# PJLab-ADG/nr3d_lib

Hardware: AMD Instinct MI355X
Metric: Mpoints/s LoTD fwd+bwd (16-lvl hash) + Mrays/s march+composite, 1 & 8 GPU (higher is better)
Workload: dtype f32; 1 GPU; configs[1]: 16-level Hash LoTD (gen_ngp_cfg: T=2^19, F=2, 6 Dense + 10 Hash), 2^20 points/GPU, fwd(+dy/dx) + dL/dx + dL/dparam, fp32; points_per_gpu=1048576, n_params=12131648, parallelism=single GPU

## Files before the change

include/nr3d_hip.h:

```cpp
#ifndef NR3D_HIP_H
#define NR3D_HIP_H
#include <stdint.h>

#ifdef __cplusplus
extern "C" {
#endif

enum { NR3D_F32 = 0, NR3D_F16 = 1, NR3D_F64 = 2, NR3D_I32 = 3, NR3D_I64 = 4, NR3D_U8 = 5, NR3D_I16 = 6, NR3D_I8 = 7 };

#define NR3D_ABI_VERSION 11

const char *nr3d_last_error(void);
int nr3d_abi_version(void);

enum {
	NR3D_PROF_LOTD_FWD = 0,
	NR3D_PROF_LOTD_FWD_LDS = 1,
	NR3D_PROF_LOTD_CONTRACT_DX = 2,
	NR3D_PROF_LOTD_BIN = 3,
	NR3D_PROF_LOTD_ACCUM = 4,
	NR3D_PROF_MARCH = 5,
	NR3D_PROF_COMPOSITE_FWD = 6,
	NR3D_PROF_COMPOSITE_BWD = 7,
	NR3D_PROF_LOTD_DIRECT = 8,
	NR3D_PROF_COUNT = 9
};
void nr3d_prof_enable(uint32_t mask);
int nr3d_prof_read(int id, double *total_ms, uint32_t *n_intervals, int reset);

enum {
	NR3D_OPT_LOTD_PAIR = 0,
	NR3D_OPT_PAIR_QUAD = 1,
	NR3D_OPT_PAIR_SECOND = 2,
	NR3D_OPT_PAIR_DIRECT = 3,
	NR3D_OPT_PAIR_FIXED = 4,
	NR3D_OPT_FWD_PAIRLANE = 5,
	NR3D_OPT_FWD_SPLIT = 6,
	NR3D_OPT_FWD_LDS_STAGE = 7,
	NR3D_OPT_HVP_LEVELS = 8,
	NR3D_OPT_HVP_PAIRLANE = 9,
	NR3D_OPT_HVP_SPLIT = 10,
	NR3D_OPT_VM_SPLIT = 11,
	NR3D_OPT_CP_DIRECT = 12,
	NR3D_OPT_MARCH_GROUP = 13,
	NR3D_OPT_PACK_SCAN = 14,
	NR3D_OPT_VM_LINES_DIRECT = 15,
	NR3D_OPT_FWD_CELL_MAJOR = 16,
	NR3D_OPT_SORT_WAVE = 17,
	NR3D_OPT_VM_DIRECT = 18,
	NR3D_OPT_DIRECT_FIXED = 19,
	NR3D_OPT_VM_SORTED = 20,
	NR3D_OPT_MLP_X3 = 21,
	NR3D_OPT_COUNT = 22
};
int nr3d_set_option(int id, int64_t value);
int64_t nr3d_get_option(int id);

#define NR3D_LOTD_MAX_LEVELS 32
#define NR3D_LOTD_MAX_DIMS 4
#define NR3D_LOTD_MAX_PSEUDO 256

enum {
	NR3D_LOD_Dense = 0, NR3D_LOD_VectorMatrix = 1, NR3D_LOD_VecZMatXoY = 2, NR3D_LOD_CP = 3,
	NR3D_LOD_CPfast = 4, NR3D_LOD_NPlaneMul = 5, NR3D_LOD_NPlaneSum = 6, NR3D_LOD_Hash = 7
};

typedef struct nr3d_lotd_level {
	uint32_t res[NR3D_LOTD_MAX_DIMS];
	uint32_t n_feats;
	uint32_t type;
	uint32_t size;
	uint32_t offset;
} nr3d_lotd_level_t;

typedef struct nr3d_lotd_meta {
	nr3d_lotd_level_t levels[NR3D_LOTD_MAX_LEVELS];
	uint16_t map_levels[NR3D_LOTD_MAX_PSEUDO];
	uint16_t map_cnt[NR3D_LOTD_MAX_PSEUDO];
	uint32_t n_levels;
	uint32_t n_pseudo_levels;
	uint32_t n_feat_per_pseudo_lvl;
	uint32_t n_dims_to_encode;
	uint32_t n_encoded_dims;
	uint32_t n_params;
	uint32_t interpolation_type;
	uint32_t c_hash_only;
	uint16_t map_col[NR3D_LOTD_MAX_PSEUDO];
} nr3d_lotd_meta_t;

int nr3d_lotd_meta_create(int32_t n_input_dim, uint32_t n_levels, const int32_t *res_multidim,
                          const int32_t *n_feats, const int32_t *types, uint32_t hashmap_size,
                          int use_smooth_step, nr3d_lotd_meta_t *out);

int nr3d_lotd_meta_regroup(const nr3d_lotd_meta_t *meta, uint32_t width, uint32_t max_width, nr3d_lotd_meta_t *out);


int nr3d_lotd_fwd(const nr3d_lotd_meta_t *meta, const void *meta_dev, uint32_t n_points,
                  int x_dtype, int param_dtype, const void *x, const void *params,
                  const int64_t *batch_inds, const int64_t *batch_offsets, uint32_t batch_data_size,
                  int32_t max_level, void *y, int64_t y_sn, int64_t y_se,
                  void *dy_dx, int64_t dydx_sn, int64_t dydx_se, void *stream);

int nr3d_lotd_bwd_dx(const nr3d_lotd_meta_t *meta, uint32_t n_points, int x_dtype, int param_dtype,
                     const void *dL_dy, int64_t dldy_sn, int64_t dldy_se,
                     const void *dy_dx, int64_t dydx_sn, int64_t dydx_se, void *dL_dx,
                     void *dL_dy_T ,
                     void *stream);

uint64_t nr3d_lotd_dparam_workspace_bytes(const nr3d_lotd_meta_t *meta, uint32_t n_points, uint32_t n_batches);
void nr3d_lotd_set_dparam_chunk_log2(int log2_points);
int nr3d_lotd_bwd_dparam(const nr3d_lotd_meta_t *meta, const void *meta_dev, uint32_t n_points,
                         int x_dtype, int param_dtype, const void *dL_dy, int64_t dldy_sn, int64_t dldy_se,
                         const void *x, const void *params, const int64_t *batch_inds,
                         const int64_t *batch_offsets, uint32_t batch_data_size, uint32_t n_batches, int32_t max_level,
                         void *dL_dparam, void *workspace, uint64_t workspace_bytes, void *stream);
int nr3d_lotd_bwd_dparam_levels(const nr3d_lotd_meta_t *meta, const void *meta_dev, uint32_t n_points,
                                int x_dtype, int param_dtype, const void *dL_dy, int64_t dldy_sn, int64_t dldy_se,
                                const void *x, const void *params, const int64_t *batch_inds,
                                const int64_t *batch_offsets, uint32_t batch_data_size, uint32_t n_batches,
                                int32_t min_level, int32_t max_level, void *dL_dparam, void *workspace,
                                uint64_t workspace_bytes, void *stream);

int nr3d_lotd_dLdy_feature_major(uint32_t n_points, uint32_t n_encoded_dims, int grad_dtype, const void *dL_dy,
                                 int64_t g_sn, int64_t g_se, float *out, void *stream);

int nr3d_lotd_half_params_ok(const nr3d_lotd_meta_t *meta, int batched);
int nr3d_lotd_pair_path_ok(const nr3d_lotd_meta_t *meta);
int nr3d_lotd_pair_direct_levels(const nr3d_lotd_meta_t *meta, uint32_t n_points);
uint64_t nr3d_lotd_fwd_lds_levels(const nr3d_lotd_meta_t *meta, uint32_t n_points, uint64_t *by_slab);
int nr3d_lotd_bwd_dparam_typed(const nr3d_lotd_meta_t *meta, const void *meta_dev, uint32_t n_points, int grad_dtype,
                               const void *dL_dy, int64_t g_sn, int64_t g_se, const void *x, int32_t max_level,
                               int out_dtype, int assign, void *dL_dparam, void *workspace, uint64_t workspace_bytes,
                               void *stream);

int nr3d_lotd_bwd_bwd_ddLdy(const nr3d_lotd_meta_t *meta, uint32_t n_points, int x_dtype, int param_dtype,
                            const void *dL_ddLdx, const void *dy_dx, int64_t dydx_sn, int64_t dydx_se,
                            void *dL_ddLdy, int64_t out_sn, int64_t out_se, void *stream);
int nr3d_lotd_bwd_bwd_dparam(const nr3d_lotd_meta_t *meta, const void *meta_dev, uint32_t n_points,
                             int x_dtype, int param_dtype, const void *dL_ddLdx,
                             const void *dL_dy, int64_t dldy_sn, int64_t dldy_se, const void *x,
                             const void *params, const int64_t *batch_inds, const int64_t *batch_offsets,
                             uint32_t batch_data_size, uint32_t n_batches, int32_t max_level, void *dL_dparam,
                             void *workspace, uint64_t workspace_bytes, void *stream);
int nr3d_lotd_bwd_bwd_dx(const nr3d_lotd_meta_t *meta, const void *meta_dev, uint32_t n_points,
                         int x_dtype, int param_dtype, const void *dL_ddLdx,
                         const void *dL_dy, int64_t dldy_sn, int64_t dldy_se, const void *x,
                         const void *params, const int64_t *batch_inds, const int64_t *batch_offsets,
                         uint32_t batch_data_size, int32_t max_level, void *dL_dx, void *stream);
uint64_t nr3d_lotd_bwd_bwd_dx_workspace_bytes(const nr3d_lotd_meta_t *meta, uint32_t n_points);
int nr3d_lotd_bwd_bwd_dx_ws(const nr3d_lotd_meta_t *meta, const void *meta_dev, uint32_t n_points,
                            int x_dtype, int param_dtype, const void *dL_ddLdx,
                            const void *dL_dy, int64_t dldy_sn, int64_t dldy_se, const void *x,
                            const void *params, const int64_t *batch_inds, const int64_t *batch_offsets,
                            uint32_t batch_data_size, int32_t max_level, void *dL_dx, void *workspace,
                            uint64_t workspace_bytes, void *stream);

int nr3d_lotd_grid_index(const nr3d_lotd_meta_t *meta, const void *meta_dev, uint32_t n_points, int x_dtype,
                         const void *x, const int64_t *batch_inds, const int64_t *batch_offsets,
                         uint32_t batch_data_size, int32_t max_level, int64_t *grid_inds, void *stream);

typedef struct nr3d_forest_meta {
	const uint8_t *octree;
	const int32_t *exsum;
	const int16_t *block_ks;
	float world_block_size[3];
	float world_origin[3];
	int32_t resolution[3];
	uint32_t n_trees;
	uint32_t level;
	uint32_t level_poffset;
	int32_t continuity_enabled;
} nr3d_forest_meta_t;

int nr3d_forest_identify(const nr3d_forest_meta_t *forest, uint64_t n, const int16_t *ks, int32_t *block_inds,
                         void *stream);

int nr3d_lotd_forest_fwd(const nr3d_lotd_meta_t *meta, const void *meta_dev, const nr3d_forest_meta_t *forest,
                         uint32_t n_points, const float *x, const void *params, int param_dtype ,
                         const int64_t *block_inds,
                         const int64_t *block_offsets, uint32_t batch_data_size, int32_t max_level, float *y,
                         int64_t y_sn, int64_t y_se, float *dy_dx, int64_t d_sn, int64_t d_se, void *stream);

uint64_t nr3d_lotd_forest_dparam_workspace_bytes(const nr3d_lotd_meta_t *meta, uint32_t n_points, uint32_t n_trees);
int nr3d_lotd_forest_bwd_dparam(const nr3d_lotd_meta_t *meta, const void *meta_dev, const nr3d_forest_meta_t *forest,
                                uint32_t n_points, const float *dL_ddLdx, const float *dL_dy, const float *x,
                                const void *params, int param_dtype, const int64_t *block_inds, const int64_t *block_offsets,
// ... 255 lines not shown
```

nr3d_lib_amd/_abi.py:

```python
ABI_VERSION = 11
SIGNATURES = {
    'nr3d_abi_version': ('int', []),
    'nr3d_alpha_to_vw_backward': ('int', ['uint32_t', 'uint64_t', 'ptr', 'ptr', 'ptr', 'ptr', 'float', 'float', 'ptr', 'ptr']),
    'nr3d_alpha_to_vw_forward': ('int', ['uint32_t', 'uint64_t', 'ptr', 'ptr', 'float', 'float', 'ptr', 'ptr', 'ptr', 'ptr']),
    'nr3d_arange_num_steps': ('int', ['uint32_t', 'int', 'ptr', 'ptr', 'ptr', 'double', 'ptr', 'ptr']),
    'nr3d_forest_identify': ('int', ['ptr', 'uint64_t', 'ptr', 'ptr', 'ptr']),
    'nr3d_forest_ray_marching_count': ('int', ['ptr', 'uint32_t', 'ptr', 'ptr', 'ptr', 'ptr', 'ptr', 'ptr', 'ptr', 'ptr', 'ptr', 'ptr', 'float', 'float', 'float', 'uint32_t', 'ptr', 'ptr', 'ptr', 'ptr']),
    'nr3d_forest_ray_marching_emit': ('int', ['ptr', 'uint32_t', 'ptr', 'ptr', 'ptr', 'ptr', 'ptr', 'ptr', 'ptr', 'ptr', 'ptr', 'ptr', 'float', 'float', 'float', 'ptr', 'ptr', 'ptr', 'ptr', 'ptr', 'ptr', 'ptr']),
    'nr3d_get_option': ('int64_t', ['int']),
    'nr3d_interleave_linstep': ('int', ['uint32_t', 'int', 'ptr', 'ptr', 'ptr', 'double', 'double', 'ptr', 'ptr', 'ptr']),
    'nr3d_last_error': ('str', []),
    'nr3d_lotd_bwd_bwd_ddLdy': ('int', ['ptr', 'uint32_t', 'int', 'int', 'ptr', 'ptr', 'int64_t', 'int64_t', 'ptr', 'int64_t', 'int64_t', 'ptr']),
    'nr3d_lotd_bwd_bwd_dparam': ('int', ['ptr', 'ptr', 'uint32_t', 'int', 'int', 'ptr', 'ptr', 'int64_t', 'int64_t', 'ptr', 'ptr', 'ptr', 'ptr', 'uint32_t', 'uint32_t', 'int32_t', 'ptr', 'ptr', 'uint64_t', 'ptr']),
    'nr3d_lotd_bwd_bwd_dx': ('int', ['ptr', 'ptr', 'uint32_t', 'int', 'int', 'ptr', 'ptr', 'int64_t', 'int64_t', 'ptr', 'ptr', 'ptr', 'ptr', 'uint32_t', 'int32_t', 'ptr', 'ptr']),
    'nr3d_lotd_bwd_bwd_dx_workspace_bytes': ('uint64_t', ['ptr', 'uint32_t']),
    'nr3d_lotd_bwd_bwd_dx_ws': ('int', ['ptr', 'ptr', 'uint32_t', 'int', 'int', 'ptr', 'ptr', 'int64_t', 'int64_t', 'ptr', 'ptr', 'ptr', 'ptr', 'uint32_t', 'int32_t', 'ptr', 'ptr', 'uint64_t', 'ptr']),
    'nr3d_lotd_bwd_dparam': ('int', ['ptr', 'ptr', 'uint32_t', 'int', 'int', 'ptr', 'int64_t', 'int64_t', 'ptr', 'ptr', 'ptr', 'ptr', 'uint32_t', 'uint32_t', 'int32_t', 'ptr', 'ptr', 'uint64_t', 'ptr']),
    'nr3d_lotd_bwd_dparam_levels': ('int', ['ptr', 'ptr', 'uint32_t', 'int', 'int', 'ptr', 'int64_t', 'int64_t', 'ptr', 'ptr', 'ptr', 'ptr', 'uint32_t', 'uint32_t', 'int32_t', 'int32_t', 'ptr', 'ptr', 'uint64_t', 'ptr']),
    'nr3d_lotd_bwd_dparam_typed': ('int', ['ptr', 'ptr', 'uint32_t', 'int', 'ptr', 'int64_t', 'int64_t', 'ptr', 'int32_t', 'int', 'int', 'ptr', 'ptr', 'uint64_t', 'ptr']),
    'nr3d_lotd_bwd_dx': ('int', ['ptr', 'uint32_t', 'int', 'int', 'ptr', 'int64_t', 'int64_t', 'ptr', 'int64_t', 'int64_t', 'ptr', 'ptr', 'ptr']),
    'nr3d_lotd_dLdy_feature_major': ('int', ['uint32_t', 'uint32_t', 'int', 'ptr', 'int64_t', 'int64_t', 'ptr', 'ptr']),
    'nr3d_lotd_dparam_workspace_bytes': ('uint64_t', ['ptr', 'uint32_t', 'uint32_t']),
    'nr3d_lotd_forest_bwd_bwd_dx': ('int', ['ptr', 'ptr', 'ptr', 'uint32_t', 'ptr', 'ptr', 'ptr', 'ptr', 'int', 'ptr', 'ptr', 'uint32_t', 'int32_t', 'ptr', 'ptr']),
    'nr3d_lotd_forest_bwd_dparam': ('int', ['ptr', 'ptr', 'ptr', 'uint32_t', 'ptr', 'ptr', 'ptr', 'ptr', 'int', 'ptr', 'ptr', 'uint32_t', 'int32_t', 'ptr', 'ptr', 'uint64_t', 'ptr']),
    'nr3d_lotd_forest_dparam_workspace_bytes': ('uint64_t', ['ptr', 'uint32_t', 'uint32_t']),
    'nr3d_lotd_forest_fwd': ('int', ['ptr', 'ptr', 'ptr', 'uint32_t', 'ptr', 'ptr', 'int', 'ptr', 'ptr', 'uint32_t', 'int32_t', 'ptr', 'int64_t', 'int64_t', 'ptr', 'int64_t', 'int64_t', 'ptr']),
    'nr3d_lotd_fwd': ('int', ['ptr', 'ptr', 'uint32_t', 'int', 'int', 'ptr', 'ptr', 'ptr', 'ptr', 'uint32_t', 'int32_t', 'ptr', 'int64_t', 'int64_t', 'ptr', 'int64_t', 'int64_t', 'ptr']),
    'nr3d_lotd_fwd_lds_levels': ('uint64_t', ['ptr', 'uint32_t', 'ptr']),
    'nr3d_lotd_grid_index': ('int', ['ptr', 'ptr', 'uint32_t', 'int', 'ptr', 'ptr', 'ptr', 'uint32_t', 'int32_t', 'ptr', 'ptr']),
    'nr3d_lotd_half_params_ok': ('int', ['ptr', 'int']),
    'nr3d_lotd_meta_create': ('int', ['int32_t', 'uint32_t', 'ptr', 'ptr', 'ptr', 'uint32_t', 'int', 'ptr']),
    'nr3d_lotd_meta_regroup': ('int', ['ptr', 'uint32_t', 'uint32_t', 'ptr']),
    'nr3d_lotd_mlp_forward': ('int', ['ptr', 'ptr', 'uint64_t', 'ptr', 'ptr', 'int', 'int32_t', 'ptr', 'ptr', 'ptr', 'int64_t', 'uint32_t', 'ptr']),
    'nr3d_lotd_mlp_forward_ok': ('int', ['ptr', 'ptr']),
    'nr3d_lotd_pair_direct_levels': ('int', ['ptr', 'uint32_t']),
    'nr3d_lotd_pair_path_ok': ('int', ['ptr']),
    'nr3d_lotd_set_dparam_chunk_log2': ('void', ['int']),
    'nr3d_march_composite_bwd': ('int', ['uint32_t', 'ptr', 'ptr', 'ptr', 'ptr', 'ptr', 'float', 'float', 'int', 'ptr', 'ptr', 'ptr', 'ptr', 'ptr', 'ptr', 'ptr', 'ptr', 'ptr', 'ptr', 'uint64_t', 'ptr', 'ptr']),
    'nr3d_march_composite_fwd': ('int', ['uint32_t', 'ptr', 'ptr', 'ptr', 'ptr', 'ptr', 'ptr', 'ptr', 'int', 'float', 'float', 'float', 'uint32_t', 'ptr', 'ptr', 'ptr', 'ptr', 'ptr', 'ptr', 'uint64_t', 'uint64_t', 'ptr', 'ptr', 'ptr', 'ptr', 'ptr', 'ptr', 'ptr', 'ptr', 'uint64_t', 'ptr', 'float', 'float', 'int', 'ptr', 'ptr', 'ptr', 'ptr', 'ptr', 'ptr']),
    'nr3d_march_finish_rays': ('int', ['uint32_t', 'ptr', 'ptr', 'ptr', 'ptr', 'ptr', 'ptr']),
    'nr3d_march_finish_samples': ('int', ['uint64_t', 'ptr', 'ptr', 'ptr', 'ptr', 'ptr', 'ptr', 'ptr', 'ptr', 'ptr']),
    'nr3d_mark_pack_boundaries': ('int', ['uint64_t', 'int', 'ptr', 'ptr', 'ptr']),
    'nr3d_merge_pack_union': ('int', ['uint32_t', 'ptr', 'ptr', 'uint32_t', 'ptr', 'ptr', 'ptr', 'ptr', 'ptr', 'ptr', 'ptr', 'ptr', 'ptr', 'ptr', 'ptr', 'ptr']),
    'nr3d_mlp_backward': ('int', ['ptr', 'uint64_t', 'ptr', 'int64_t', 'int64_t', 'ptr', 'int64_t', 'ptr', 'ptr', 'int64_t', 'int64_t', 'ptr', 'ptr', 'ptr']),
    'nr3d_mlp_backward_backward': ('int', ['ptr', 'uint64_t', 'ptr', 'int64_t', 'int64_t', 'ptr', 'int64_t', 'ptr', 'int64_t', 'int64_t', 'ptr', 'ptr', 'int64_t', 'ptr', 'ptr']),
    'nr3d_mlp_backward_backward_ok': ('int', ['ptr']),
    'nr3d_mlp_backward_packed_floats': ('uint64_t', ['ptr']),
    'nr3d_mlp_forward': ('int', ['ptr', 'uint64_t', 'ptr', 'int64_t', 'int64_t', 'ptr', 'ptr', 'int64_t', 'ptr']),
    'nr3d_mlp_half_backward': ('int', ['ptr', 'uint64_t', 'ptr', 'int64_t', 'int64_t', 'ptr', 'int64_t', 'ptr', 'ptr', 'int64_t', 'int64_t', 'ptr', 'ptr', 'ptr']),
    'nr3d_mlp_half_backward_packed_bytes': ('uint64_t', ['ptr']),
    'nr3d_mlp_half_forward': ('int', ['ptr', 'uint64_t', 'ptr', 'int64_t', 'int64_t', 'ptr', 'ptr', 'int64_t', 'ptr']),
    'nr3d_mlp_half_pack': ('int', ['ptr', 'ptr', 'ptr', 'ptr', 'int', 'ptr']),
    'nr3d_mlp_half_packed_bytes': ('uint64_t', ['ptr']),
    'nr3d_mlp_pack': ('int', ['ptr', 'ptr', 'ptr', 'ptr', 'int', 'ptr']),
    'nr3d_mlp_packed_floats': ('uint64_t', ['ptr']),
    'nr3d_occ_apply_max': ('int', ['uint64_t', 'float', 'ptr', 'ptr', 'ptr']),
    'nr3d_occ_scatter_max': ('int', ['uint64_t', 'ptr', 'ptr', 'ptr', 'uint64_t', 'ptr', 'ptr', 'uint32_t', 'ptr', 'ptr']),
    'nr3d_octree_mark_consecutive_segments': ('int', ['uint32_t', 'ptr', 'ptr', 'ptr', 'ptr', 'ptr', 'ptr']),
    'nr3d_order_gather_inputs': ('int', ['uint32_t', 'ptr', 'ptr', 'ptr', 'ptr', 'ptr', 'ptr', 'ptr', 'ptr']),
    'nr3d_order_move_rows': ('int', ['uint32_t', 'ptr', 'int', 'ptr', 'uint32_t', 'ptr', 'ptr', 'uint32_t', 'ptr', 'ptr']),
    'nr3d_pack_composite_bwd': ('int', ['uint32_t', 'ptr', 'ptr', 'ptr', 'ptr', 'ptr', 'ptr', 'float', 'float', 'int', 'ptr', 'ptr', 'ptr', 'ptr', 'ptr', 'ptr', 'ptr', 'ptr', 'ptr', 'ptr']),
    'nr3d_pack_composite_fwd': ('int', ['uint32_t', 'ptr', 'ptr', 'ptr', 'ptr', 'ptr', 'float', 'float', 'int', 'ptr', 'ptr', 'ptr', 'ptr', 'ptr']),
    'nr3d_pack_infos_from_n': ('int', ['uint32_t', 'ptr', 'ptr', 'ptr', 'ptr', 'ptr']),
    'nr3d_packed_binary': ('int', ['uint32_t', 'uint64_t', 'uint32_t', 'uint32_t', 'int', 'ptr', 'ptr', 'ptr', 'int', 'int', 'ptr', 'ptr']),
    'nr3d_packed_diff': ('int', ['uint32_t', 'uint64_t', 'uint32_t', 'int', 'ptr', 'ptr', 'ptr', 'ptr', 'int', 'int', 'ptr', 'ptr']),
    'nr3d_packed_invert_cdf': ('int', ['uint32_t', 'ptr', 'ptr', 'ptr', 'ptr', 'uint32_t', 'ptr', 'ptr', 'ptr']),
    'nr3d_packed_scan': ('int', ['uint32_t', 'uint64_t', 'uint32_t', 'int', 'ptr', 'ptr', 'int', 'int', 'int', 'int', 'ptr', 'ptr']),
    'nr3d_packed_searchsorted': ('int', ['uint32_t', 'int', 'ptr', 'ptr', 'ptr', 'uint32_t', 'ptr', 'ptr', 'ptr']),
    'nr3d_packed_sort': ('int', ['uint32_t', 'uint64_t', 'int', 'ptr', 'ptr', 'ptr', 'ptr']),
    'nr3d_packed_sum': ('int', ['uint32_t', 'uint64_t', 'uint32_t', 'int', 'ptr', 'ptr', 'ptr', 'ptr']),
    'nr3d_permuto_bwd': ('int', ['ptr', 'uint32_t', 'int', 'ptr', 'int64_t', 'int64_t', 'ptr', 'ptr', 'ptr', 'ptr', 'ptr', 'ptr', 'uint32_t', 'int32_t', 'uint32_t', 'ptr', 'ptr', 'ptr']),
    'nr3d_permuto_bwd_bwd_input': ('int', ['ptr', 'uint32_t', 'int', 'ptr', 'ptr', 'int64_t', 'int64_t', 'ptr', 'ptr', 'ptr', 'ptr', 'ptr', 'ptr', 'uint32_t', 'int32_t', 'ptr', 'int64_t', 'int64_t', 'ptr', 'ptr']),
    'nr3d_permuto_fwd': ('int', ['ptr', 'uint32_t', 'int', 'ptr', 'ptr', 'ptr', 'ptr', 'ptr', 'ptr', 'uint32_t', 'int32_t', 'ptr', 'int64_t', 'int64_t', 'ptr']),
    'nr3d_permuto_meta_create': ('int', ['int32_t', 'int32_t', 'uint32_t', 'ptr', 'ptr', 'ptr', 'ptr']),
    'nr3d_permuto_supported_n_input_dims': ('int', ['ptr']),
    'nr3d_prof_enable': ('void', ['uint32_t']),
    'nr3d_prof_read': ('int', ['int', 'ptr', 'ptr', 'int']),
    'nr3d_prune_compact_packs': ('int', ['uint32_t', 'ptr', 'ptr', 'ptr', 'ptr', 'ptr', 'ptr', 'ptr', 'ptr']),
    'nr3d_prune_compact_samples': ('int', ['uint32_t', 'ptr', 'ptr', 'ptr', 'ptr', 'ptr', 'ptr', 'ptr', 'ptr', 'ptr', 'ptr', 'ptr', 'ptr', 'ptr']),
    'nr3d_ray_marching_cache_bytes': ('uint64_t', ['uint32_t', 'uint32_t']),
    'nr3d_ray_marching_count': ('int', ['uint32_t', 'ptr', 'ptr', 'ptr', 'ptr', 'ptr', 'ptr', 'ptr', 'int', 'float', 'float', 'float', 'uint32_t', 'int', 'ptr', 'uint32_t', 'ptr', 'ptr', 'ptr', 'ptr', 'uint64_t', 'ptr']),
    'nr3d_ray_marching_count_finished': ('int', ['uint32_t', 'ptr', 'ptr', 'ptr', 'ptr', 'ptr', 'ptr', 'ptr', 'int', 'float', 'float', 'float', 'uint32_t', 'int', 'ptr', 'uint32_t', 'ptr', 'ptr', 'ptr', 'ptr', 'ptr', 'ptr', 'uint64_t', 'ptr']),
    'nr3d_ray_marching_emit': ('int', ['uint32_t', 'ptr', 'ptr', 'ptr', 'ptr', 'ptr', 'ptr', 'ptr', 'int', 'float', 'float', 'float', 'int', 'ptr', 'uint32_t', 'ptr', 'ptr', 'ptr', 'ptr', 'ptr', 'ptr', 'ptr', 'uint32_t', 'ptr']),
    'nr3d_ray_marching_emit_finished': ('int', ['uint32_t', 'ptr', 'ptr', 'int', 'ptr', 'uint32_t', 'ptr', 'ptr', 'uint32_t', 'ptr', 'ptr', 'ptr', 'ptr', 'ptr', 'ptr', 'ptr', 'ptr', 'ptr']),
    'nr3d_sample_step_count': ('int', ['uint32_t', 'ptr', 'ptr', 'uint32_t', 'float', 'float', 'float', 'ptr', 'ptr']),
    'nr3d_sample_step_emit': ('int', ['uint32_t', 'ptr', 'ptr', 'float', 'float', 'float', 'ptr', 'ptr', 'ptr', 'ptr']),
    'nr3d_sample_step_segments': ('int', ['uint32_t', 'ptr', 'ptr', 'ptr', 'ptr', 'ptr', 'uint32_t', 'float', 'float', 'float', 'int', 'ptr', 'ptr', 'ptr', 'ptr', 'ptr', 'ptr', 'ptr']),
    'nr3d_scan_tmp_bytes': ('uint64_t', ['uint64_t']),
# ... 11 lines not shown
```

nr3d_lib_amd/_hip.py:

```python
import ctypes as C
import os
import subprocess
import threading

import torch

from nr3d_lib_amd import _abi

_PKG = os.path.dirname(os.path.abspath(__file__))
LIB_PATH = os.path.join(_PKG, "libnr3d_hip.so")
ABI_VERSION = _abi.ABI_VERSION
CSRC = os.path.join(_PKG, "csrc")

F32, F16, F64, I32, I64, U8, I16, I8 = range(8)
DTYPE_CODE = {
    torch.float32: F32, torch.float16: F16, torch.float64: F64, torch.int32: I32, torch.int64: I64,
    torch.uint8: U8, torch.bool: U8, torch.int16: I16, torch.int8: I8,
}

_lib = None
_lock = threading.Lock()


def build(verbose=False, jobs=None):
# ... 53 lines not shown
    if missing:
        raise RuntimeError(f"nr3d_lib_amd: {LIB_PATH} does not export {missing} (stale build? `make -C nr3d_lib_amd/csrc`)")


POISON = os.environ.get("NR3D_POISON_EMPTY", "0") == "1"


def _poison(t):
    if t.numel() == 0:
        return t
    if t.dtype.is_floating_point:
        t.fill_(float("nan"))
    elif t.dtype == torch.bool:
        t.fill_(True)
    else:
        t.fill_(-0x54545455 if t.dtype in (torch.int32, torch.int64) else 0x2B)
    return t


def empty(*args, **kwargs):
    t = torch.empty(*args, **kwargs)
    return _poison(t) if POISON else t


def empty_like(x, **kwargs):
    t = torch.empty_like(x, **kwargs)
    return _poison(t) if POISON else t


def check(rc):
    if rc != 0:
        raise RuntimeError(lib().nr3d_last_error().decode())


PROF_IDS = dict(lotd_fwd=0, lotd_fwd_lds=1, lotd_contract_dx=2, lotd_bin=3, lotd_accum=4, march=5, composite_fwd=6,
                composite_bwd=7, lotd_direct=8)


def prof_enable(*names):
    mask = 0
    for n in names:
        mask |= 1 << PROF_IDS[n]
    lib().nr3d_prof_enable(C.c_uint32(mask))


def prof_read(name, reset=True):
    ms, n = C.c_double(0.0), C.c_uint32(0)
    check(lib().nr3d_prof_read(C.c_int(PROF_IDS[name]), C.byref(ms), C.byref(n), C.c_int(1 if reset else 0)))
    return float(ms.value), int(n.value)


OPTION_IDS = dict(lotd_pair=0, pair_quad=1, pair_second=2, pair_direct=3, pair_fixed=4, fwd_pairlane=5, fwd_split=6,
                  fwd_lds_stage=7, hvp_levels=8, hvp_pairlane=9, hvp_split=10, vm_split=11, cp_direct=12, march_group=13,
                  pack_scan=14, vm_lines_direct=15, fwd_cell_major=16, sort_wave=17, vm_direct=18, direct_fixed=19, vm_sorted=20, mlp_x3=21)


def set_option(name, value):
    l = lib()
    check(l.nr3d_set_option(OPTION_IDS[name], -1 if value is None else int(value)))


def get_option(name):
    l = lib()
    return int(l.nr3d_get_option(OPTION_IDS[name]))


class options:

    def __init__(self, **kw):
        self.kw, self.old = kw, {}

    def __enter__(self):
        for k, v in self.kw.items():
            self.old[k] = get_option(k)
            set_option(k, v)
        return self

    def __exit__(self, *a):
        for k, v in self.old.items():
            set_option(k, v)
        return False


def ptr(t):
    if t is None:
        return None
    return t.data_ptr()


_raw_stream = getattr(torch._C, "_cuda_getCurrentRawStream", None)


def stream_of(t):
    if _raw_stream is not None:
        return _raw_stream(t.device.index if t.device.index is not None else torch.cuda.current_device())
    return torch.cuda.current_stream(t.device).cuda_stream


def sort_pairs_u32(keys, values=None, bits=32, n_dev=None):
    pair = isinstance(keys, (list, tuple))
    ks = list(keys) if pair else [keys]
    vs = list(values) if isinstance(values, (list, tuple)) else [values] * len(ks)
    assert len(ks) in (1, 2) and all(k.is_cuda and k.dtype == torch.int32 and k.is_contiguous() and k.shape == ks[0].shape for k in ks)
    assert all(v is None or (v.is_cuda and v.dtype == torch.int32 and v.is_contiguous() and v.shape == ks[0].shape) for v in vs)
    n, dev = ks[0].numel(), ks[0].device
    l = lib()
    l.nr3d_sort_pairs_u32_tmp_bytes.restype = C.c_uint64
# ... 160 lines not shown
```

nr3d_lib_amd/bindings/_lotd.py:

```python
import ctypes as C
import enum

import torch

from .. import _hip as H

MAX_LEVELS, MAX_DIMS, MAX_PSEUDO = 32, 4, 256


class LoDType(enum.IntEnum):
    Dense = 0
    VectorMatrix = 1
    VecZMatXoY = 2
    CP = 3
    CPfast = 4
    NPlaneMul = 5
    NPlaneSum = 6
    Hash = 7


class InterpolationType(enum.IntEnum):
    Linear = 0
    Smoothstep = 1

# ... 345 lines not shown
                                              H.F16 if native else H.F32, max_level, C.byref(mlp_desc._c), H.ptr(mlp_packed), H.ptr(out),
                                              out_cols, out_cols, H.stream_of(input)))
    return out


def lod_bwd(lod_meta, dL_dy, input, params, dy_dx=None, batch_inds=None, batch_offsets=None, batch_data_size=None,
            max_level=None, need_input_grad=None, need_param_grad=None, level_buckets=None, on_bucket=None):
    if isinstance(lod_meta, tuple):
        from . import _forest
        return _forest.lod_bwd(lod_meta, dL_dy, input, params, dy_dx, batch_inds, batch_offsets, batch_data_size, max_level,
                               need_input_grad, need_param_grad)
    m = lod_meta
    N, bds = _check_common("bwd", m, input, params, batch_inds, batch_offsets, batch_data_size)
    E, D = m.n_encoded_dims, m.n_dims_to_encode
    H.require_gpu(dL_dy, dy_dx)
    if dL_dy.dim() != 2 or tuple(dL_dy.shape) != (N, E):
        raise RuntimeError(f"bwd: Expected dL_dy of size [{N}, {E}], got {list(dL_dy.shape)}")
    if dL_dy.dtype != params.dtype:
        raise RuntimeError("bwd: Expected dL_dy and grid to have the same dtype")
    if dy_dx is not None and dy_dx.dtype != input.dtype:
        raise RuntimeError("bwd: Expected x and dy_dx to have the same dtype")
    max_level = m.n_levels if max_level is None else int(max_level)
    need_input_grad = bool(input.requires_grad) if need_input_grad is None else bool(need_input_grad)
    need_param_grad = bool(params.requires_grad) if need_param_grad is None else bool(need_param_grad)
    dev = input.device
    dL_dx = dL_dparam = None
    with H.on_device(dev):
        if need_input_grad and dy_dx is None:
            raise RuntimeError("LoTDEncoding::bwd: need `dy_dx` to comput `dL_dx`.")
        batched = batch_inds is not None or batch_offsets is not None or bds != 0
        nothing = max_level <= -1 or not (need_input_grad or need_param_grad) or N == 0
        native = (_native_half(m, params, batched) and level_buckets is None and USE_BINNED_DPARAM and input.dtype == torch.float32
                  and dL_dy.is_contiguous() and E % 4 == 0 and dL_dy.data_ptr() % 8 == 0 and not nothing
                  and params.shape[0] == m.n_params)
        typed = (not nothing and not batched and level_buckets is None and USE_BINNED_DPARAM
                 and (native or params.dtype == torch.float32) and params.shape[0] == m.n_params
                 and bool(H.lib().nr3d_lotd_pair_path_ok(C.byref(m._cmeta()))))
        if need_input_grad:
            dL_dx = (torch.zeros if nothing else H.empty)((N, D), dtype=torch.float32, device=dev)
        if need_param_grad:
            dL_dparam = (H.empty if typed else torch.zeros)((params.shape[0],), dtype=torch.float16 if native else torch.float32,
                                                                device=dev)
        if nothing:
            if need_param_grad and level_buckets is not None and on_bucket is not None:
                for k, (lo, hi) in enumerate(level_buckets):
                    on_bucket(k, dL_dparam[m.level_offsets[int(lo)]:m.level_offsets[min(int(hi), m.n_levels - 1) + 1]])
            return (_cast(dL_dx, input.dtype), _cast(dL_dparam, params.dtype))
        g32 = dL_dy.detach() if native else _f32c(dL_dy.detach())
        gcode = H.F16 if native else H.F32
        gsn, gse = _strides2(g32)
        st = H.stream_of(input)
        tag = ("dx" if need_input_grad else "") + ("dp" if need_param_grad else "")
        with _Prof(m, f"LoTD{D}-bwd-{tag}", N):
            gT = None
            if need_input_grad and N > 0:
                j, jsn, jse = _jac_view(dy_dx.detach(), N, E, D)
                if (need_param_grad and not batched and USE_BINNED_DPARAM and gse == 1 and gsn == E
                        and g32.data_ptr() % 16 == 0):
                    gT = H.empty((E, N), dtype=torch.float32, device=dev)
                H.check(H.lib().nr3d_lotd_bwd_dx(
                    C.byref(m._cmeta()), H.u32(N), C.c_int(H.F32), C.c_int(gcode), H.ptr(g32), H.i64(gsn),
                    H.i64(gse), H.ptr(j), H.i64(jsn), H.i64(jse), H.ptr(dL_dx), H.ptr(gT), st))
            if need_param_grad and N > 0 and typed:
                ws, wsb = _dparam_workspace(m, N, dev, 1)
                if gT is not None:
                    g32, gsn, gse, gcode = gT, 1, N, H.F32
                H.check(H.lib().nr3d_lotd_bwd_dparam_typed(
                    C.byref(m._cmeta()), H.ptr(m._dev(dev)), H.u32(N), C.c_int(gcode), H.ptr(g32), H.i64(gsn), H.i64(gse),
                    H.ptr(_f32c(input.detach())), H.i32(max_level), C.c_int(H.F16 if native else H.F32), C.c_int(1),
                    H.ptr(dL_dparam), H.ptr(ws), C.c_uint64(wsb), st))
            elif need_param_grad and N > 0:
                x32, (p32, pcode) = _f32c(input.detach()), _ptab(params)
                nbat = _n_batches(m, p32, batch_offsets, batched)
                ws, wsb = _dparam_workspace(m, N, dev, nbat)
                if gT is not None:
                    g32, gsn, gse = gT, 1, N
                if level_buckets is None:
                    H.check(H.lib().nr3d_lotd_bwd_dparam(
                        C.byref(m._cmeta()), H.ptr(m._dev(dev)), H.u32(N), C.c_int(H.F32), C.c_int(pcode),
                        H.ptr(g32), H.i64(gsn), H.i64(gse), H.ptr(x32), H.ptr(p32), H.ptr(batch_inds),
                        H.ptr(batch_offsets), H.u32(bds), H.u32(nbat), H.i32(max_level), H.ptr(dL_dparam), H.ptr(ws),
                        C.c_uint64(wsb), st))
                else:
                    if batched:
                        raise RuntimeError("bwd: level_buckets need non-batched params")
                    if params.dtype != torch.float32:
                        raise RuntimeError("bwd: level_buckets need float params (the slices handed out are the result)")
                    seen = set()
                    for k, (lo, hi) in enumerate(level_buckets):
                        lo, hi = int(lo), min(int(hi), m.n_levels - 1)
                        if lo < 0 or lo > hi or seen & set(range(lo, hi + 1)):
                            raise RuntimeError(f"bwd: bad or overlapping level bucket {(lo, hi)}")
                        seen |= set(range(lo, hi + 1))
                        H.check(H.lib().nr3d_lotd_bwd_dparam_levels(
                            C.byref(m._cmeta()), H.ptr(m._dev(dev)), H.u32(N), C.c_int(H.F32), C.c_int(H.F32),
                            H.ptr(g32), H.i64(gsn), H.i64(gse), H.ptr(x32), H.ptr(p32), None, None, H.u32(0),
                            H.u32(nbat), H.i32(lo), H.i32(min(hi, max_level)), H.ptr(dL_dparam), H.ptr(ws),
                            C.c_uint64(wsb), st))
                        if on_bucket is not None:
                            on_bucket(k, dL_dparam[m.level_offsets[lo]:m.level_offsets[hi + 1]])
    return _cast(dL_dx, input.dtype), _cast(dL_dparam, params.dtype)


def _cast(t, dtype):
    if t is None or t.dtype == dtype:
        return t
    return t.to(dtype)


def lod_bwd_bwd_input(lod_meta, dL_ddLdx, dL_dy, input, params, dy_dx=None, batch_inds=None, batch_offsets=None,
                      batch_data_size=None, max_level=None, need_dLdinput_ddLdoutput=None,
                      need_dLdinput_dparams=None, need_dLdinput_dinput=None):
    if isinstance(lod_meta, tuple):
        from . import _forest
        return _forest.lod_bwd_bwd_input(lod_meta, dL_ddLdx, dL_dy, input, params, dy_dx, batch_inds, batch_offsets,
                                         batch_data_size, max_level, need_dLdinput_ddLdoutput, need_dLdinput_dparams,
                                         need_dLdinput_dinput)
    m = lod_meta
    N, bds = _check_common("bwd_bwd_input", m, input, params, batch_inds, batch_offsets, batch_data_size)
    E, D = m.n_encoded_dims, m.n_dims_to_encode
    H.require_gpu(dL_ddLdx, dL_dy, dy_dx)
    if input.dtype != torch.float32:
        raise RuntimeError("LoTDEncoding: Input type combination not supported. Supported types are: "
# ... 87 lines not shown
```

nr3d_lib_amd/csrc/host_api.hip:

```cpp
#include "common.h"
#include <stdlib.h>
#include <utility>
#include <string.h>
#include <limits>
#include <chrono>
#include <mutex>
#include <vector>

namespace nr3d {

static thread_local char g_err[512] = {0};

char *err_buf() { return g_err; }

int fail(const char *fmt, ...) {
	va_list ap;
	va_start(ap, fmt);
	vsnprintf(g_err, sizeof(g_err), fmt, ap);
	va_end(ap);
	return 1;
}

namespace prof {
uint32_t g_mask = 0;
struct Pair { hipEvent_t a, b; };
static std::mutex g_mu;
static std::vector<Pair> g_done[NR3D_PROF_COUNT];
static std::vector<Pair> g_free;
static Pair g_open[NR3D_PROF_COUNT];
static bool g_is_open[NR3D_PROF_COUNT] = {};

void begin(int id, hipStream_t st) {
	std::lock_guard<std::mutex> lk(g_mu);
	if (id < 0 || id >= NR3D_PROF_COUNT || g_is_open[id]) return;
	Pair p;
	if (!g_free.empty()) { p = g_free.back(); g_free.pop_back(); }
	else if (hipEventCreate(&p.a) != hipSuccess || hipEventCreate(&p.b) != hipSuccess) return;
	if (hipEventRecord(p.a, st) != hipSuccess) return;
	g_open[id] = p; g_is_open[id] = true;
}
void end(int id, hipStream_t st) {
	std::lock_guard<std::mutex> lk(g_mu);
	if (id < 0 || id >= NR3D_PROF_COUNT || !g_is_open[id]) return;
	g_is_open[id] = false;
	if (hipEventRecord(g_open[id].b, st) == hipSuccess) g_done[id].push_back(g_open[id]);
}
}

namespace opt {
static const int64_t kDefault[NR3D_OPT_COUNT] = {
	 1,  1,  1,  1,  1,  1,
	 1,  1,  1,  1,  1,  1,
	 1,  0,  1,  0,  1,  1,
	 1,  1,  1,  1,
};
std::atomic<int64_t> g_val[NR3D_OPT_COUNT] = {1, 1, 1, 1, 1, 1, 1, 1, 1, 1, 1, 1, 1, 0, 1, 0, 1, 1, 1, 1, 1, 1};

#ifdef NR3D_EXPERIMENTS
int64_t experiment_env(const char *name, int64_t dflt) {
	static std::mutex mu;
	static std::vector<std::pair<const char *, int64_t>> seen;
	std::lock_guard<std::mutex> lk(mu);
	for (const auto &kv : seen) if (kv.first == name) return kv.second;
	const char *e = getenv(name);
	const int64_t v = e ? (int64_t)atoll(e) : dflt;
	seen.emplace_back(name, v);
	return v;
}
#endif
}

}

using namespace nr3d;

extern "C" void nr3d_prof_enable(uint32_t mask) { prof::g_mask = mask; }

extern "C" int nr3d_prof_read(int id, double *total_ms, uint32_t *n_intervals, int reset) {
	NR3D_CHECK(id >= 0 && id < NR3D_PROF_COUNT && total_ms && n_intervals, "prof_read: bad argument");
	std::lock_guard<std::mutex> lk(prof::g_mu);
	double sum = 0.0;
	for (const prof::Pair &p : prof::g_done[id]) {
		NR3D_HIP_CHECK(hipEventSynchronize(p.b));
		float ms = 0.0f;
		NR3D_HIP_CHECK(hipEventElapsedTime(&ms, p.a, p.b));
		sum += ms;
	}
	*total_ms = sum;
	*n_intervals = (uint32_t)prof::g_done[id].size();
	if (reset) {
		for (const prof::Pair &p : prof::g_done[id]) prof::g_free.push_back(p);
		prof::g_done[id].clear();
	}
	return 0;
}

extern "C" int nr3d_set_option(int id, int64_t value) {
	NR3D_CHECK(id >= 0 && id < NR3D_OPT_COUNT, "nr3d_set_option: unknown option %d", id);
	opt::g_val[id].store(value < 0 ? opt::kDefault[id] : value, std::memory_order_relaxed);
	return 0;
}
extern "C" int64_t nr3d_get_option(int id) { return (id >= 0 && id < NR3D_OPT_COUNT) ? opt::get(id) : -1; }

extern "C" int nr3d_wait_host_words(const int64_t *words, int n, int64_t sentinel, uint32_t timeout_us) {
	if (!words || n <= 0) return 0;
	const auto t0 = std::chrono::steady_clock::now();
	for (uint32_t spin = 0;; ++spin) {
		bool all = true;
		for (int i = 0; i < n; ++i)
// ... 136 lines not shown
```

nr3d_lib_amd/csrc/lotd.hip:

```cpp
#include "lotd_device.h"
#include <stdlib.h>
#include <vector>
#include <type_traits>
#include <algorithm>

namespace nr3d {
namespace lotd {

template <typename YT> __device__ __forceinline__ void store_nt(YT *p, float v);

template <int D, int G, bool DYDX, bool DH, int ONLY = -1, typename PT = float>
__global__ __launch_bounds__(kBlock) void k_fwd(Sched s, const nr3d_lotd_meta_t *__restrict__ md, uint32_t N,
                                                int32_t max_level, uint32_t smooth, const float *__restrict__ x,
                                                const PT *__restrict__ params, Batch ba, uint32_t vec_ok,
                                                PT *__restrict__ y, int64_t y_sn, int64_t y_se,
                                                float *__restrict__ dydx, int64_t d_sn, int64_t d_se) {
	uint32_t q, chunk;
	if (!decode_block(s, blockIdx.x, q, chunk)) return;
	const uint32_t i = chunk * kBlock + threadIdx.x;
	if (i >= N) return;
	const uint32_t level = meta_level_of(md, q);
	const uint32_t foff0 = meta_cnt_of(md, q) * G;
	const uint32_t out0 = meta_col_of(md, q);

// ... 1149 lines not shown
		if (side == 0u && g0 + pl < N) {
			float *dst = reinterpret_cast<float *>(reinterpret_cast<char *>(partial) + ((size_t)q * N + g0) * 12u + pl * 12u);
			__builtin_nontemporal_store(ox[u], &dst[0]);
			__builtin_nontemporal_store(oy[u], &dst[1]);
			__builtin_nontemporal_store(oz[u], &dst[2]);
		}
	}
}

template <int D>
__global__ __launch_bounds__(kBlock) void k_sum_levels(uint32_t N, uint32_t n_pseudo, const float *__restrict__ partial,
                                                       float *__restrict__ dL_dx) {
	const uint32_t i = blockIdx.x * kBlock + threadIdx.x;
	if (i >= N) return;
	float acc[D];
#pragma unroll
	for (int d = 0; d < D; ++d) acc[d] = 0.0f;
	for (uint32_t q = 0; q < n_pseudo; ++q) {
		const float *src = partial + ((size_t)q * N + i) * D;
#pragma unroll
		for (int d = 0; d < D; ++d) acc[d] += __builtin_nontemporal_load(src + d);
	}
#pragma unroll
	for (int d = 0; d < D; ++d) dL_dx[(size_t)i * D + d] = acc[d];
}


template <int D>
__global__ __launch_bounds__(kBlock) void k_contract_dx(uint32_t N, uint32_t E, const float *__restrict__ dL_dy,
                                                        int64_t g_sn, int64_t g_se, const float *__restrict__ dydx,
                                                        int64_t d_sn, int64_t d_se, float *__restrict__ dL_dx) {
	const uint32_t i = blockIdx.x * kBlock + threadIdx.x;
	if (i >= N) return;
	float acc[D];
#pragma unroll
	for (int d = 0; d < D; ++d) acc[d] = 0.0f;
	const float *gy = dL_dy + (int64_t)i * g_sn;
	const float *jj = dydx + (int64_t)i * d_sn;
#pragma unroll 4
	for (uint32_t e = 0; e < E; ++e) {
		const float g = gy[(int64_t)e * g_se];
		const float *j = jj + (int64_t)e * d_se;
#pragma unroll
		for (int d = 0; d < D; ++d) acc[d] = __fmaf_rn(g, j[d], acc[d]);
	}
#pragma unroll
	for (int d = 0; d < D; ++d) dL_dx[(size_t)i * D + d] = acc[d];
}

template <int D, typename GT>
__global__ __launch_bounds__(kBlock) void k_contract_dx_rowmajor(uint32_t N, uint32_t E, const GT *__restrict__ dL_dy,
                                                                 const float *__restrict__ dydx, int64_t d_sn,
                                                                 int64_t d_se, float *__restrict__ dL_dx,
                                                                 float *__restrict__ dL_dy_T) {
	constexpr int TE = 32;
	__shared__ float tile[TE][kBlock + 1];
	const uint32_t i0 = blockIdx.x * kBlock, i = i0 + threadIdx.x;
	const uint32_t n_here = min((uint32_t)kBlock, N - i0);
	float acc[D];
#pragma unroll
	for (int d = 0; d < D; ++d) acc[d] = 0.0f;
	for (uint32_t e0 = 0; e0 < E; e0 += TE) {
		const uint32_t te = min((uint32_t)TE, E - e0);
		if (te == TE && (E & 3u) == 0u) {
#pragma unroll
			for (uint32_t v = threadIdx.x; v < kBlock * TE / 4; v += kBlock) {
				const uint32_t p = v >> 3, e4 = (v & 7u) * 4u;
				if (p < n_here) {
					float4 t;
					if constexpr (sizeof(GT) == 4) {
						t = *reinterpret_cast<const float4 *>(dL_dy + (size_t)(i0 + p) * E + e0 + e4);
					} else {
						const __half2 *h = reinterpret_cast<const __half2 *>(dL_dy + (size_t)(i0 + p) * E + e0 + e4);
						const float2 a = __half22float2(h[0]), b = __half22float2(h[1]);
						t = make_float4(a.x, a.y, b.x, b.y);
					}
					tile[e4][p] = t.x; tile[e4 + 1][p] = t.y; tile[e4 + 2][p] = t.z; tile[e4 + 3][p] = t.w;
				}
			}
		} else {
			for (uint32_t v = threadIdx.x; v < kBlock * te; v += kBlock) {
				const uint32_t p = v / te, e = v - p * te;
				if (p < n_here) tile[e][p] = to_f32<GT>(dL_dy[(size_t)(i0 + p) * E + e0 + e]);
			}
		}
		__syncthreads();
		if (dL_dy_T && i < N) {
#pragma unroll 8
			for (uint32_t e = 0; e < te; ++e) __builtin_nontemporal_store(tile[e][threadIdx.x], &dL_dy_T[(size_t)(e0 + e) * N + i]);
		}
		if (i < N) {
			const float *jj = dydx + (int64_t)i * d_sn + (int64_t)e0 * d_se;
#pragma unroll 8
			for (uint32_t e = 0; e < te; ++e) {
				const float g = tile[e][threadIdx.x];
				const float *j = jj + (int64_t)e * d_se;
#pragma unroll
				for (int d = 0; d < D; ++d) acc[d] = __fmaf_rn(g, __builtin_nontemporal_load(j + d), acc[d]);
			}
		}
		__syncthreads();
	}
	if (i < N) {
#pragma unroll
		for (int d = 0; d < D; ++d) dL_dx[(size_t)i * D + d] = acc[d];
	}
}

template <int D>
__global__ __launch_bounds__(kBlock) void k_contract_ddLdy(uint32_t N, uint32_t E, const float *__restrict__ v,
                                                           const float *__restrict__ dydx, int64_t d_sn, int64_t d_se,
                                                           float *__restrict__ out, int64_t o_sn, int64_t o_se) {
	const uint32_t i = blockIdx.x * kBlock + threadIdx.x;
	const uint32_t e = blockIdx.y;
	if (i >= N) return;
	const float *j = dydx + (int64_t)i * d_sn + (int64_t)e * d_se;
	float r = 0.0f;
#pragma unroll
	for (int d = 0; d < D; ++d) r = __fmaf_rn(v[(size_t)i * D + d], j[d], r);
	out[(int64_t)i * o_sn + (int64_t)e * o_se] = r;
}

template <int D, int G>
__global__ __launch_bounds__(kBlock) void k_grid_index(Sched s, const nr3d_lotd_meta_t *__restrict__ md, uint32_t N,
                                                       uint32_t E, int32_t max_level, const float *__restrict__ x,
                                                       Batch ba, int64_t *__restrict__ out) {
	uint32_t q, chunk;
	if (!decode_block(s, blockIdx.x, q, chunk)) return;
	const uint32_t i = chunk * kBlock + threadIdx.x;
	if (i >= N) return;
	const uint32_t level = meta_level_of(md, q);
	if ((int32_t)level > max_level) return;
	uint32_t base = 0;
	if (!batch_base(ba, i, base)) return;
	const Lvl L = load_level(md, level);
	const uint32_t foff0 = meta_cnt_of(md, q) * G;
	float xp[D];
#pragma unroll
	for (int d = 0; d < D; ++d) xp[d] = x[(size_t)i * D + d];
	Cell<D> c;
	locate<D>(xp, L, false, c);
	int64_t *dst = out + ((size_t)i * E + (size_t)meta_col_of(md, q)) * (1u << D);
#pragma unroll
	for (uint32_t k = 0; k < (1u << D); ++k) {
		uint32_t p[D];
		corner_pos<D>(c, k, p);
		const uint32_t e = (L.type == NR3D_LOD_Dense) ? entry_dense<D>(L, p) : entry_hash<D>(L, p);
		const uint32_t ind = base + L.off + e * L.F + foff0;
#pragma unroll
		for (int f = 0; f < G; ++f) dst[k + f * (1u << D)] = (int64_t)(uint32_t)(ind + f);
	}
}

static uint32_t sched_mode_default() { const int64_t m = NR3D_XOPT(LOTD_SCHED, 3); return (m < 0 || m > 3) ? 3u : (uint32_t)m; }
static bool sched_exclusive_enabled() { return NR3D_XOPT(LOTD_SCHED_EXCL, 1) != 0; }

static uint32_t level_cost(const nr3d_lotd_meta_t *m, uint32_t q, bool pairlane = false) {
	const nr3d_lotd_level_t &L = m->levels[m->map_levels[q]];
// ... 318 lines not shown
                       bool p_half, const int64_t *batch_inds, const int64_t *batch_offsets, uint32_t batch_data_size,
                       int32_t max_level, void *y, int64_t y_sn, int64_t y_se, void *dy_dx, int64_t d_sn, int64_t d_se,
                       hipStream_t st) {
	uint32_t n_blocks;
	const Batch ba{batch_inds, batch_offsets, batch_data_size, meta->n_params};
	const uint32_t G = meta->n_feat_per_pseudo_lvl;
	const uint32_t elt = p_half ? 2u : 4u;
	const uint32_t vec_ok = (((uintptr_t)params % ((G >= 4 ? 4u : 2u) * elt)) == 0 && batch_offsets == nullptr) ? 1u : 0u;
	const bool dh = meta->c_hash_only != 0;
	prof::Scope ps(NR3D_PROF_LOTD_FWD, st);
	uint64_t grp[4] = {0, 0, 0, 0};
	const bool split = !dh && meta->n_pseudo_levels <= 64u && opt::on(NR3D_OPT_FWD_SPLIT);
	const uint64_t all = meta->n_pseudo_levels >= 64u ? ~0ull : ((1ull << meta->n_pseudo_levels) - 1ull);
	if (split) {
		for (uint32_t q = 0; q < meta->n_pseudo_levels; ++q) {
			const uint32_t t = meta->levels[meta->map_levels[q]].type;
			int k = 0;
			if (t == NR3D_LOD_Dense || t == NR3D_LOD_Hash) k = 1;
			else if (meta->n_dims_to_encode == 3 && t == NR3D_LOD_CP) k = 2;
			else if (meta->n_dims_to_encode == 3 && t == NR3D_LOD_VectorMatrix) k = 3;
			grp[k] |= 1ull << q;
		}
	} else {
		grp[dh ? 1 : 0] = all;
	}
	for (int k = 0; k < 4; ++k) {
		if (!grp[k]) continue;
		const uint64_t skip = (split || meta->n_pseudo_levels <= 64u) ? (all & ~grp[k]) : 0ull;
		const Sched s = make_sched(N, meta, n_blocks, skip);
		if (n_blocks == 0) continue;
		DISPATCH_DG(meta->n_dims_to_encode, G, {
			auto launch = [&](auto kern_f32, auto kern_f16) {
				if (p_half)
					hipLaunchKernelGGL(kern_f16, dim3(n_blocks), dim3(kBlock), 0, st, s, md, N, max_level,
					                   meta->interpolation_type, (const float *)x, (const __half *)params, ba, vec_ok,
					                   (__half *)y, y_sn, y_se, (float *)dy_dx, d_sn, d_se);
				else
					hipLaunchKernelGGL(kern_f32, dim3(n_blocks), dim3(kBlock), 0, st, s, md, N, max_level,
					                   meta->interpolation_type, (const float *)x, (const float *)params, ba, vec_ok,
					                   (float *)y, y_sn, y_se, (float *)dy_dx, d_sn, d_se);
			};
			if (k == 1) { if (dy_dx) NR3D_FWD2(D, true, true, -1); else NR3D_FWD2(D, false, true, -1); }
			else if (k == 0) { if (dy_dx) NR3D_FWD2(D, true, false, -1); else NR3D_FWD2(D, false, false, -1); }
			else if constexpr (D == 3) {
				if (k == 2) { if (dy_dx) NR3D_FWD2(3, true, false, NR3D_LOD_CP); else NR3D_FWD2(3, false, false, NR3D_LOD_CP); }
				else { if (dy_dx) NR3D_FWD2(3, true, false, NR3D_LOD_VectorMatrix); else NR3D_FWD2(3, false, false, NR3D_LOD_VectorMatrix); }
			}
		});
	}
	NR3D_LAUNCH_CHECK();
	return 0;
}

extern "C" int nr3d_lotd_bwd_dx(const nr3d_lotd_meta_t *meta, uint32_t N, int x_dtype, int param_dtype,
                                const void *dL_dy, int64_t g_sn, int64_t g_se, const void *dy_dx, int64_t d_sn,
                                int64_t d_se, void *dL_dx, void *dL_dy_T, void *stream) {
	NR3D_CHECK(meta != nullptr, "LoTD: meta is NULL");
	NR3D_CHECK(x_dtype == NR3D_F32 && (param_dtype == NR3D_F32 || param_dtype == NR3D_F16), "LoTD::bwd_dx: f32 x, f32 / f16 dL_dy");
	if (N == 0) return 0;
	NR3D_CHECK(dL_dy && dy_dx && dL_dx, "LoTDEncoding::bwd: need `dy_dx` to comput `dL_dx`.");
	const uint32_t E = meta->n_encoded_dims;
	const bool g_half = param_dtype == NR3D_F16;
	const bool row_major = (g_se == 1 && g_sn == (int64_t)E && ((uintptr_t)dL_dy % (g_half ? 8 : 16)) == 0);
	NR3D_CHECK(dL_dy_T == nullptr || row_major, "LoTD::bwd_dx: dL_dy_T needs a contiguous, 16-byte aligned [N, E] dL_dy");
	NR3D_CHECK(!g_half || (row_major && (E & 3u) == 0u), "LoTD::bwd_dx: half dL_dy must be a contiguous [N, E] tensor, E % 4 == 0");
	prof::Scope ps(NR3D_PROF_LOTD_CONTRACT_DX, (hipStream_t)stream);
	DISPATCH_D(meta->n_dims_to_encode, {
		if (row_major && g_half)
			hipLaunchKernelGGL((k_contract_dx_rowmajor<D, __half>), dim3(div_up(N, kBlock)), dim3(kBlock), 0, (hipStream_t)stream, N, E,
			                   (const __half *)dL_dy, (const float *)dy_dx, d_sn, d_se, (float *)dL_dx, (float *)dL_dy_T);
		else if (row_major)
			hipLaunchKernelGGL((k_contract_dx_rowmajor<D, float>), dim3(div_up(N, kBlock)), dim3(kBlock), 0, (hipStream_t)stream, N, E,
			                   (const float *)dL_dy, (const float *)dy_dx, d_sn, d_se, (float *)dL_dx, (float *)dL_dy_T);
		else
			hipLaunchKernelGGL(k_contract_dx<D>, dim3(div_up(N, kBlock)), dim3(kBlock), 0, (hipStream_t)stream, N, E,
			                   (const float *)dL_dy, g_sn, g_se, (const float *)dy_dx, d_sn, d_se, (float *)dL_dx);
	});
	NR3D_LAUNCH_CHECK();
	return 0;
}

static int launch_bwd_dparam(bool second, const nr3d_lotd_meta_t *meta, const void *meta_dev, uint32_t N,
                             const void *dL_ddLdx, const void *dL_dy, int64_t g_sn, int64_t g_se, const void *x,
                             const void *params, const int64_t *batch_inds, const int64_t *batch_offsets,
                             uint32_t batch_data_size, uint32_t n_batches, int32_t max_level, void *dL_dparam,
                             void *workspace, uint64_t workspace_bytes, void *stream, int32_t min_level = 0, bool p_half = false) {
	if (N == 0 || max_level <= -1 || min_level > max_level) return 0;
	NR3D_CHECK(dL_dy && x && params && dL_dparam, "LoTD::bwd: NULL tensor pointer");
	const bool batched = batch_inds || batch_offsets || batch_data_size;
	if (workspace && (!batched || n_batches > 0)) {
		bool handled = false;
		const Batch bb{batch_inds, batch_offsets, batch_data_size, meta->n_params};
		if (int rc = dparam_binned(second, meta, meta_dev, N, (const float *)dL_ddLdx, (const float *)dL_dy, g_sn, g_se,
		                           (const float *)x, (const float *)params, bb, batched ? n_batches : 1u, max_level,
		                           (float *)dL_dparam, workspace, workspace_bytes, (hipStream_t)stream, handled, nullptr,
		                           min_level, false, false, false, p_half))
			return rc;
		if (handled) return 0;
	}
	uint32_t n_blocks;
	const Sched s = make_sched(N, meta, n_blocks);
	const Batch ba{batch_inds, batch_offsets, batch_data_size, meta->n_params};
	const auto md = (const nr3d_lotd_meta_t *)meta_dev;
	const bool dh = meta->c_hash_only != 0;
	DISPATCH_DG(meta->n_dims_to_encode, meta->n_feat_per_pseudo_lvl, {
		auto launch = [&](auto kern, auto *tab) {
			hipLaunchKernelGGL(kern, dim3(n_blocks), dim3(kBlock), 0, (hipStream_t)stream, s, md, N, min_level, max_level,
			                   meta->interpolation_type, (const float *)dL_ddLdx, (const float *)dL_dy, g_sn, g_se,
			                   (const float *)x, tab, ba, (float *)dL_dparam);
		};
		const float *pf = (const float *)params;
		const __half *ph = (const __half *)params;
		if (dh || !p_half) {
			if (second) { if (dh) launch(k_bwd_dparam<D, G, true, true>, pf); else launch(k_bwd_dparam<D, G, true, false>, pf); }
			else        { if (dh) launch(k_bwd_dparam<D, G, false, true>, pf); else launch(k_bwd_dparam<D, G, false, false>, pf); }
		} else {
			if (second) launch(k_bwd_dparam<D, G, true, false, __half>, ph); else launch(k_bwd_dparam<D, G, false, false, __half>, ph);
		}
	});
	NR3D_LAUNCH_CHECK();
	return 0;
}

extern "C" int nr3d_lotd_bwd_dparam(const nr3d_lotd_meta_t *meta, const void *meta_dev, uint32_t N, int x_dtype,
                                    int param_dtype, const void *dL_dy, int64_t g_sn, int64_t g_se, const void *x,
                                    const void *params, const int64_t *batch_inds, const int64_t *batch_offsets,
                                    uint32_t batch_data_size, uint32_t n_batches, int32_t max_level, void *dL_dparam,
                                    void *workspace, uint64_t workspace_bytes, void *stream) {
	if (int rc = check_common(meta, meta_dev, x_dtype, param_dtype, true)) return rc;
	return launch_bwd_dparam(false, meta, meta_dev, N, nullptr, dL_dy, g_sn, g_se, x, params, batch_inds,
	                         batch_offsets, batch_data_size, n_batches, max_level, dL_dparam, workspace, workspace_bytes,
	                         stream, 0, param_dtype == NR3D_F16);
}

extern "C" int nr3d_lotd_pair_path_ok(const nr3d_lotd_meta_t *meta) { return (meta && pair_applies(meta)) ? 1 : 0; }
extern "C" uint64_t nr3d_lotd_fwd_lds_levels(const nr3d_lotd_meta_t *meta, uint32_t n_points, uint64_t *by_slab) {
	if (by_slab) *by_slab = 0;
	if (!meta || !pairlane_enabled() || !pairlane_meta_ok(meta)) return 0;
	return fwd_lds_levels(meta, n_points, 0x7fffffff, by_slab);
}

extern "C" int nr3d_lotd_pair_direct_levels(const nr3d_lotd_meta_t *meta, uint32_t n_points) {
	return (meta && pair_applies(meta)) ? (int)pair_direct_levels(meta, n_points) : 0;
}

extern "C" int nr3d_lotd_bwd_dparam_typed(const nr3d_lotd_meta_t *meta, const void *meta_dev, uint32_t N, int grad_dtype,
                                          const void *dL_dy, int64_t g_sn, int64_t g_se, const void *x, int32_t max_level,
                                          int out_dtype, int assign, void *dL_dparam, void *workspace, uint64_t workspace_bytes,
                                          void *stream) {
	if (int rc = check_common(meta, meta_dev, NR3D_F32, NR3D_F32)) return rc;
	NR3D_CHECK((grad_dtype == NR3D_F32 || grad_dtype == NR3D_F16) && (out_dtype == NR3D_F32 || out_dtype == NR3D_F16),
	           "LoTD::bwd_dparam_typed: f32 / f16 only");
	if (N == 0 || max_level <= -1) {
		if (assign && dL_dparam)
			NR3D_HIP_CHECK(hipMemsetAsync(dL_dparam, 0, (size_t)meta->n_params * (out_dtype == NR3D_F16 ? 2 : 4), (hipStream_t)stream));
		return 0;
	}
	NR3D_CHECK(dL_dy && x && dL_dparam && workspace, "LoTD::bwd: NULL tensor pointer");
	bool handled = false;
	const Batch bb{nullptr, nullptr, 0u, meta->n_params};
	if (int rc = dparam_binned(false, meta, meta_dev, N, nullptr, (const float *)dL_dy, g_sn, g_se, (const float *)x, nullptr, bb,
	                           1u, max_level, (float *)dL_dparam, workspace, workspace_bytes, (hipStream_t)stream, handled, nullptr,
	                           0, grad_dtype == NR3D_F16, out_dtype == NR3D_F16, assign != 0))
		return rc;
	NR3D_CHECK(handled, "LoTD::bwd_dparam_typed: the pair-record path does not apply to this meta / workspace");
	return 0;
}

extern "C" int nr3d_lotd_bwd_dparam_levels(const nr3d_lotd_meta_t *meta, const void *meta_dev, uint32_t N, int x_dtype,
                                           int param_dtype, const void *dL_dy, int64_t g_sn, int64_t g_se, const void *x,
                                           const void *params, const int64_t *batch_inds, const int64_t *batch_offsets,
                                           uint32_t batch_data_size, uint32_t n_batches, int32_t min_level,
                                           int32_t max_level, void *dL_dparam, void *workspace, uint64_t workspace_bytes,
                                           void *stream) {
	if (int rc = check_common(meta, meta_dev, x_dtype, param_dtype, true)) return rc;
	NR3D_CHECK(min_level >= 0, "LoTD::bwd: min_level must be >= 0");
	return launch_bwd_dparam(false, meta, meta_dev, N, nullptr, dL_dy, g_sn, g_se, x, params, batch_inds,
	                         batch_offsets, batch_data_size, n_batches, max_level, dL_dparam, workspace, workspace_bytes,
	                         stream, min_level, param_dtype == NR3D_F16);
}

extern "C" void nr3d_lotd_set_dparam_chunk_log2(int log2_points) { set_dparam_chunk_log2(log2_points); }

extern "C" uint64_t nr3d_lotd_dparam_workspace_bytes(const nr3d_lotd_meta_t *meta, uint32_t n_points, uint32_t n_batches) {
	return dparam_workspace_bytes(meta, n_points, n_batches);
}

extern "C" int nr3d_lotd_bwd_bwd_dparam(const nr3d_lotd_meta_t *meta, const void *meta_dev, uint32_t N, int x_dtype,
                                        int param_dtype, const void *dL_ddLdx, const void *dL_dy, int64_t g_sn,
                                        int64_t g_se, const void *x, const void *params, const int64_t *batch_inds,
                                        const int64_t *batch_offsets, uint32_t batch_data_size, uint32_t n_batches,
                                        int32_t max_level, void *dL_dparam, void *workspace, uint64_t workspace_bytes,
                                        void *stream) {
	if (int rc = check_common(meta, meta_dev, x_dtype, param_dtype, true)) return rc;
	NR3D_CHECK(N == 0 || dL_ddLdx != nullptr, "LoTD::bwd_bwd_input: dL_ddLdx is NULL");
	return launch_bwd_dparam(true, meta, meta_dev, N, dL_ddLdx, dL_dy, g_sn, g_se, x, params, batch_inds,
	                         batch_offsets, batch_data_size, n_batches, max_level, dL_dparam, workspace, workspace_bytes,
	                         stream, 0, param_dtype == NR3D_F16);
}

extern "C" int nr3d_lotd_bwd_bwd_ddLdy(const nr3d_lotd_meta_t *meta, uint32_t N, int x_dtype, int param_dtype,
                                       const void *dL_ddLdx, const void *dy_dx, int64_t d_sn, int64_t d_se,
                                       void *dL_ddLdy, int64_t o_sn, int64_t o_se, void *stream) {
	NR3D_CHECK(meta != nullptr, "LoTD: meta is NULL");
	NR3D_CHECK(x_dtype == NR3D_F32 && param_dtype == NR3D_F32, "LoTD::bwd_bwd_ddLdy: f32 only");
	if (N == 0) return 0;
	NR3D_CHECK(dL_ddLdx && dy_dx && dL_ddLdy, "LoTDEncoding::bwd_bwd_input: need `dy_dx` to compute `dL_d(dLdy)`.");
	DISPATCH_D(meta->n_dims_to_encode, {
		hipLaunchKernelGGL(k_contract_ddLdy<D>, dim3(div_up(N, kBlock), meta->n_encoded_dims), dim3(kBlock), 0,
		                   (hipStream_t)stream, N, meta->n_encoded_dims, (const float *)dL_ddLdx,
		                   (const float *)dy_dx, d_sn, d_se, (float *)dL_ddLdy, o_sn, o_se);
	});
	NR3D_LAUNCH_CHECK();
	return 0;
}

template <typename PT>
static int launch_bwd_bwd_dx_t(const nr3d_lotd_meta_t *meta, const void *meta_dev, uint32_t N, int x_dtype, int param_dtype,
                             const void *dL_ddLdx, const void *dL_dy, int64_t g_sn, int64_t g_se, const void *x,
// ... 141 lines not shown
```

nr3d_lib_amd/csrc/lotd_bin.hip:

```cpp
#include "lotd_vm.h"
#include "lotd_sorted.h"
#include <stdlib.h>
#include <type_traits>

#ifndef NR3D_BIN_LDS_KB
#define NR3D_BIN_LDS_KB 72
#define NR3D_BIN_MAX_BP 512
#endif
namespace nr3d {
namespace lotd {

constexpr int kAccThreads = 1024;
constexpr int kLdsDoubles = 16384;
constexpr int kRedSlots = 4;
#ifndef NR3D_BALLOT_RANK_BUCKETS
#define NR3D_BALLOT_RANK_BUCKETS 4
#endif
constexpr uint32_t kBallotRankBuckets = NR3D_BALLOT_RANK_BUCKETS;
constexpr int kMaxPlanLevels = 64;
constexpr uint32_t kMaxBuckets = 8192;
constexpr int kBinLdsDyn = NR3D_BIN_LDS_KB * 1024 + (int)(kMaxBuckets + 1) * 4;

#define DISPATCH_DG_BIN(D_, G_, ...)                                                 \
	do {                                                                             \
// ... 881 lines not shown
		p[k] = flush_target<G>(plan, L, ba, foff0, b, (row0 + (uint32_t)k) * kAccThreads + threadIdx.x, dparam, slot[k]);
		if (!p[k]) slot[k] = 0;
		sum[k] = 0.0f;
	}
#pragma unroll
	for (int k = 0; k < NS; ++k) old[k] = p[k] ? *p[k] : 0.0f;
	for (uint32_t r0 = 0; r0 < R; r0 += NR) {
		float v[NS][NR];
#pragma unroll
		for (int k = 0; k < NS; ++k)
#pragma unroll
			for (int j = 0; j < NR; ++j) v[k][j] = (r0 + j < R) ? part0[(size_t)(r0 + j) * kLdsDoubles + slot[k]] : 0.0f;
#pragma unroll
		for (int k = 0; k < NS; ++k)
#pragma unroll
			for (int j = 0; j < NR; ++j) sum[k] += v[k][j];
	}
#pragma unroll
	for (int k = 0; k < NS; ++k) if (p[k]) *p[k] = old[k] + sum[k];
}

template <int D, int G>
__global__ __launch_bounds__(kAccThreads) void k_reduce_partials(BinPlan plan, const nr3d_lotd_meta_t *__restrict__ md,
                                                                 const uint32_t *__restrict__ rep_g,
                                                                 const uint32_t *__restrict__ item_start, Batch ba,
                                                                 const float *__restrict__ partial,
                                                                 float *__restrict__ dparam) {
	const uint32_t fb = blockIdx.x;
	const uint32_t R = rep_g[fb];
	if (R <= 1) return;
	const bool wide = R <= 4;
	if (wide && blockIdx.y >= kLdsDoubles / kAccThreads / kRedSlots) return;
	uint32_t q = 0;
	while (q + 1 < plan.n_pseudo && plan.bucket_base[q + 1] <= fb) ++q;
	const uint32_t b = fb - plan.bucket_base[q], qg = plan.qmap[q];
	const Lvl L = load_level(md, meta_level_of(md, qg));
	const uint32_t foff0 = meta_cnt_of(md, qg) * G;
	const float *part0 = partial + (size_t)item_start[fb] * kLdsDoubles;
	if (wide) reduce_rows<G, kRedSlots, 4>(plan, L, ba, foff0, b, R, blockIdx.y * kRedSlots, part0, dparam);
	else reduce_rows<G, 1, 8>(plan, L, ba, foff0, b, R, blockIdx.y, part0, dparam);
}

static uint32_t work_units() {
	const int64_t v = NR3D_XOPT(LOTD_ACC_UNITS, 960);
	return (uint32_t)(v < 256 ? 256 : (v > 8192 ? 8192 : v));
}

static int g_chunk_log2 = 0;
void set_dparam_chunk_log2(int lg) { g_chunk_log2 = lg <= 0 ? 0 : (lg < 10 ? 10 : (lg > 24 ? 24 : lg)); }
static uint32_t chunk_points(uint32_t n) {
	const uint32_t chunk = 1u << (g_chunk_log2 ? g_chunk_log2 : 22);
	return n < chunk ? n : chunk;
}

constexpr int kCpThreads = 1024;
constexpr uint32_t kCpMaxItems = 32, kCpLdsBytes = 144 * 1024, kCpReplicas = 128, kCpMaxPairs = 4;
struct CpPlan {
	uint32_t n_items, R, pts_per_rep;
	uint32_t q[kCpMaxItems];
	uint32_t np[kCpMaxItems];
	uint32_t part_off[kCpMaxItems];
};

template <bool SECOND, typename PT>
__global__ __launch_bounds__(kCpThreads) void k_cp_direct(CpPlan cp, const nr3d_lotd_meta_t *__restrict__ md, uint32_t n, uint32_t smooth,
                                                          const float *__restrict__ x, const float *__restrict__ vin_,
                                                          const float *__restrict__ g, int64_t g_sn, int64_t g_se,
                                                          const PT *__restrict__ params, float *__restrict__ partial, uint32_t opt_fix) {
	extern __shared__ __attribute__((aligned(16))) double cp_acc[];
	unsigned long long *cp_fix = reinterpret_cast<unsigned long long *>(cp_acc);
	__shared__ uint32_t s_bound[3];
	const uint32_t r = blockIdx.x, item = blockIdx.y;
	const uint32_t q = cp.q[item], np = cp.np[item], row = 2u * np;
	const Lvl L = load_level(md, meta_level_of(md, q));
	const uint32_t n_acc = L.size * row;
	for (uint32_t t = threadIdx.x; t < n_acc; t += kCpThreads) cp_acc[t] = 0.0;
	if (threadIdx.x < 3) s_bound[threadIdx.x] = 0u;
	__syncthreads();
	const uint32_t foff = meta_cnt_of(md, q) * 2u, col0 = meta_col_of(md, q);
	const auto grid = make_tab(params + L.off + foff);
	const bool vec = (tab_addr(grid) % (2u * tab_elt(grid))) == 0u && (L.F & 1u) == 0u;
	const bool quad = (tab_addr(grid) % (4u * tab_elt(grid))) == 0u && (L.F & 3u) == 0u;
	const uint32_t p_lo = r * cp.pts_per_rep, p_hi = min(n, p_lo + cp.pts_per_rep);
	{
		uint32_t gb = 0u, pb = 0u, vb = 0u;
		for (uint32_t i = p_lo + threadIdx.x; i < p_hi; i += kCpThreads) {
			for (uint32_t f = 0; f < row; ++f) gb = max(gb, __float_as_uint(g[(int64_t)i * g_sn + (int64_t)(col0 + f) * g_se]) & 0x7FFFFFFFu);
			if (SECOND)
#pragma unroll
				for (int d = 0; d < 3; ++d) vb = max(vb, __float_as_uint(vin_[(size_t)i * 3 + d]) & 0x7FFFFFFFu);
		}
		for (uint32_t t = threadIdx.x; t < n_acc; t += kCpThreads)
			pb = max(pb, __float_as_uint((float)grid[(t / row) * L.F + (t % row)]) & 0x7FFFFFFFu);
#pragma unroll
		for (int off = 32; off >= 1; off >>= 1) {
			gb = max(gb, (uint32_t)__shfl_xor((int)gb, off, 64)); pb = max(pb, (uint32_t)__shfl_xor((int)pb, off, 64));
			vb = max(vb, (uint32_t)__shfl_xor((int)vb, off, 64));
		}
		if ((threadIdx.x & 63u) == 0u) { atomicMax(&s_bound[0], gb); atomicMax(&s_bound[1], pb); atomicMax(&s_bound[2], vb); }
	}
	__syncthreads();
	double fscale = 0.0, finv = 0.0;
	bool fix = false;
	{
		const float gmax = __uint_as_float(s_bound[0]), pmax = __uint_as_float(s_bound[1]), vmax = __uint_as_float(s_bound[2]);
		float B = gmax * pmax * pmax;
// ... 514 lines not shown
				hipLaunchKernelGGL((k_bin<D, G, false, NR, false, __half>), dim3(pl.n_blk, pl.n_pseudo), dim3(BP), bin_lds, st, pl, md, n, max_level,
				                   meta->interpolation_type, xc, vc, gc, sn, se, (const __half *)params_, ba, rec, offs);
		}
	} else if (second)
		hipLaunchKernelGGL((k_bin<D, G, true, NR, DH>), dim3(pl.n_blk, pl.n_pseudo), dim3(BP), bin_lds, st, pl, md, n, max_level,
		                   meta->interpolation_type, xc, vc, gc, sn, se, params, ba, rec, offs);
	else
		hipLaunchKernelGGL((k_bin<D, G, false, NR, DH>), dim3(pl.n_blk, pl.n_pseudo), dim3(BP), bin_lds, st, pl, md, n, max_level,
		                   meta->interpolation_type, xc, vc, gc, sn, se, params, ba, rec, offs);
	prof::end(NR3D_PROF_LOTD_BIN, st);
	hipLaunchKernelGGL(k_bucket_totals, dim3(div_up(NB, 4)), dim3(256), 0, st, pl, offs, tot);
	hipLaunchKernelGGL(k_plan_items, dim3(1), dim3(1024), 0, st, NB, pl.n_blk, work_units(), tot, rep, item_start);
	{
		prof::Scope ps(NR3D_PROF_LOTD_ACCUM, st);
		hipLaunchKernelGGL((k_accum<D, G>), dim3(work_units() + NB), dim3(kAccThreads), kLdsDoubles * 8, st, pl, md, rec, offs, rep,
		                   item_start, ba, partial, dparam);
	}
	hipLaunchKernelGGL((k_reduce_partials<D, G>), dim3(NB, kLdsDoubles / kAccThreads), dim3(kAccThreads), 0, st, pl, md, rep, item_start, ba, partial, dparam);
	NR3D_LAUNCH_CHECK();
	return 0;
}

}
}

extern "C" int nr3d_lotd_dLdy_feature_major(uint32_t n_points, uint32_t n_encoded_dims, int grad_dtype, const void *dL_dy,
                                            int64_t g_sn, int64_t g_se, float *out, void *stream) {
	using namespace nr3d;
	using namespace nr3d::lotd;
	NR3D_CHECK(grad_dtype == NR3D_F32 || grad_dtype == NR3D_F16, "dLdy_feature_major: f32 / f16 dL_dy");
	if (n_points == 0 || n_encoded_dims == 0) return 0;
	NR3D_CHECK(dL_dy && out, "dLdy_feature_major: NULL tensor pointer");
	if (grad_dtype == NR3D_F16) launch_transpose<__half>(n_points, n_encoded_dims, (const __half *)dL_dy, g_sn, g_se, out, (hipStream_t)stream);
	else launch_transpose<float>(n_points, n_encoded_dims, (const float *)dL_dy, g_sn, g_se, out, (hipStream_t)stream);
	NR3D_LAUNCH_CHECK();
	return 0;
}

static_assert(sizeof(nr3d_lotd_meta_t) % 4 == 0 && sizeof(nr3d_lotd_meta_t) <= 3584, "the narrowed meta rides in the kernel arguments");
__global__ void k_store_meta(const nr3d_lotd_meta_t m, uint32_t *__restrict__ dst) {
	const uint32_t *src = (const uint32_t *)&m;
	for (uint32_t i = threadIdx.x; i < sizeof(nr3d_lotd_meta_t) / 4; i += blockDim.x) dst[i] = src[i];
}

namespace nr3d {
namespace lotd {

static bool pair_second_enabled() { return opt::on(NR3D_OPT_PAIR_SECOND); }

int dparam_binned(bool second, const nr3d_lotd_meta_t *meta, const void *meta_dev, uint32_t N, const float *dL_ddLdx,
                  const float *dL_dy, int64_t g_sn, int64_t g_se, const float *x, const float *params, const Batch &batch,
                  uint32_t n_batches, int32_t max_level, float *dparam, void *workspace, uint64_t workspace_bytes,
                  hipStream_t st, bool &handled, const ForestDev *forest, int32_t min_level, bool g_half, bool out_half, bool assign,
                  bool p_half) {
	handled = false;
	BinLayout lay;
	const uint32_t nc = chunk_points(N);
	nr3d_lotd_meta_t narrow;
	const bool narrowed = workspace && stage_a_meta(meta, forest != nullptr, narrow);
	if (narrowed) meta = &narrow;
	if (!workspace || !binnable(meta, forest != nullptr) || !layout(meta, nc, n_batches, lay, forest != nullptr)) return 0;
	if (workspace_bytes < lay.total + (narrowed ? kStageAMetaBytes : 0)) return 0;
	handled = true;
	if (narrowed) {
		k_store_meta<<<1, 256, 0, st>>>(narrow, (uint32_t *)((char *)workspace + lay.total));
		NR3D_HIP_CHECK(hipGetLastError());
		meta_dev = (char *)workspace + lay.total;
	}
	const auto md = (const nr3d_lotd_meta_t *)meta_dev;
	const uint32_t D = meta->n_dims_to_encode, G = meta->n_feat_per_pseudo_lvl, E = meta->n_encoded_dims;
	uint32_t *rec = (uint32_t *)workspace;
	uint32_t *offs = (uint32_t *)((char *)workspace + lay.rec_bytes);
	uint32_t *plan_buf = (uint32_t *)((char *)workspace + lay.rec_bytes + lay.offs_bytes);
	float *partial = (float *)((char *)workspace + lay.rec_bytes + lay.offs_bytes + lay.plan_bytes);
	float *gt = (float *)((char *)workspace + lay.rec_bytes + lay.offs_bytes + lay.plan_bytes + lay.part_bytes);
	const bool row_major = (g_se == 1 && g_sn == (int64_t)E && E > 1) || g_half;
	const bool use_pair = !forest && n_batches <= 1 && !batch.inds && !batch.offsets && !batch.data_size && pair_applies(meta) &&
	                      !(second && !pair_second_enabled());
	if ((g_half || out_half) && !use_pair)
		return ::nr3d::fail("LoTD::bwd: half gradients are served natively on the pair-record path only (nr3d_lotd_half_params_ok)");
	const bool assign_now = assign && use_pair && N <= nc && min_level <= 0 && max_level >= (int32_t)meta->n_levels - 1;
	if (assign && !assign_now)
		NR3D_HIP_CHECK(hipMemsetAsync(dparam, 0, (size_t)(n_batches ? n_batches : 1u) * meta->n_params * (out_half ? 2 : 4), st));

	for (uint32_t p0 = 0; p0 < N; p0 += nc) {
		const uint32_t n = (N - p0) < nc ? (N - p0) : nc;
		const float *xc = x + (size_t)p0 * D;
		const float *vc = dL_ddLdx ? dL_ddLdx + (size_t)p0 * D : nullptr;
		const float *gc = g_half ? reinterpret_cast<const float *>(reinterpret_cast<const __half *>(dL_dy) + (int64_t)p0 * g_sn)
		                         : dL_dy + (int64_t)p0 * g_sn;
		int64_t sn = g_sn, se = g_se;
		Batch ba = batch;
		if (ba.inds) ba.inds += p0;
		ba.first_point = p0;
		bool gt_ready = !row_major;
		auto need_gt = [&]() {
			if (gt_ready) return;
			if (g_half) launch_transpose<__half>(n, E, reinterpret_cast<const __half *>(gc), g_sn, g_se, gt, st);
			else launch_transpose<float>(n, E, gc, g_sn, g_se, gt, st);
			gc = gt; sn = 1; se = (int64_t)n;
			gt_ready = true;
		};
		if (use_pair) {
			need_gt();
			if (int rc = pair_chunk(meta, md, n, xc, gc, sn, se, min_level, max_level, work_units(), dparam,
			                        (out_half ? 1u : 0u) | (assign_now ? 2u : 0u), rec, offs, plan_buf, partial, st,
			                        second ? vc : nullptr))
				return rc;
			continue;
		}
		uint64_t cp_mask = 0;
		if (!forest && n_batches <= 1 && !batch.inds && !batch.offsets && !batch.data_size) {
			CpPlan cp;
			uint32_t max_acc = 0;
			cp_mask = cp_plan(meta, n, min_level, max_level, lay.part_bytes / 4, cp, max_acc);
			if (cp_mask) {
				static bool cp_attr[64] = {};
				int dev_id = 0;
				NR3D_HIP_CHECK(hipGetDevice(&dev_id));
				if (!cp_attr[dev_id & 63]) {
					NR3D_HIP_CHECK(hipFuncSetAttribute((const void *)k_cp_direct<false, float>, hipFuncAttributeMaxDynamicSharedMemorySize, (int)kCpLdsBytes));
					NR3D_HIP_CHECK(hipFuncSetAttribute((const void *)k_cp_direct<true, float>, hipFuncAttributeMaxDynamicSharedMemorySize, (int)kCpLdsBytes));
					NR3D_HIP_CHECK(hipFuncSetAttribute((const void *)k_cp_direct<false, __half>, hipFuncAttributeMaxDynamicSharedMemorySize, (int)kCpLdsBytes));
					NR3D_HIP_CHECK(hipFuncSetAttribute((const void *)k_cp_direct<true, __half>, hipFuncAttributeMaxDynamicSharedMemorySize, (int)kCpLdsBytes));
					cp_attr[dev_id & 63] = true;
				}
				need_gt();
				const size_t lds = (size_t)max_acc * 8;
				auto cp_launch = [&](auto kern, auto *tab) {
					hipLaunchKernelGGL(kern, dim3(cp.R, cp.n_items), dim3(kCpThreads), lds, st, cp, md, n, meta->interpolation_type, xc, vc,
					                   gc, sn, se, tab, partial, opt::on(NR3D_OPT_DIRECT_FIXED) ? 1u : 0u);
				};
				if (p_half) {
					if (second) cp_launch(k_cp_direct<true, __half>, (const __half *)params); else cp_launch(k_cp_direct<false, __half>, (const __half *)params);
				} else {
					if (second) cp_launch(k_cp_direct<true, float>, params); else cp_launch(k_cp_direct<false, float>, params);
				}
				hipLaunchKernelGGL(k_cp_reduce, dim3(div_up(max_acc, 256u), cp.n_items), dim3(256), 0, st, cp, md, partial, dparam);
				NR3D_LAUNCH_CHECK();
			}
		}
		if (!g_half) {
			VsPlan vsp;
			const uint64_t smask = vm_sorted_plan(meta, n, n_batches, forest != nullptr, min_level, max_level, cp_mask, vsp);
			if (smask) {
				VsScratch vss;
				vm_sorted_scratch(vsp, n, E, second, forest != nullptr, vss);
				if (vss.total <= lay.rec_bytes + lay.offs_bytes) {
					if (int rc = vm_sorted_run(second, vsp, meta, md, n, xc, vc, dL_dy + (int64_t)p0 * g_sn, g_sn, g_se, params, p_half, ba, forest, dparam,
					                           (char *)workspace, vss, st))
						return rc;
					cp_mask |= smask;
				}
			}
		}
		if (!forest && n_batches <= 1 && !batch.inds && !batch.offsets && !batch.data_size) {
			VmPlan vp;
			const uint64_t vmask = vm_direct_plan(meta, n, min_level, max_level, lay.part_bytes / 4, vp, cp_mask);
			if (vmask) {
				static bool vattr[64] = {};
// ... 137 lines not shown
```

nr3d_lib_amd/csrc/lotd_device.h:

```cpp
#pragma once
#include "common.h"

namespace nr3d {
namespace lotd {

constexpr int kBlock = 256;
constexpr uint32_t kPrimes[7] = {1u, 2654435761u, 805459861u, 3674653429u, 2097192037u, 1434869437u, 2165219737u};

constexpr int kSchedSegs = 16;
struct Sched {
	uint32_t n_chunks, n_pseudo, mode, n_slots;
	uint64_t skip;
	uint32_t seg_cum[8][kSchedSegs + 1];
	uint32_t seg_begin[8][kSchedSegs];
	uint32_t seg_q[8][kSchedSegs];
};

__device__ __forceinline__ bool decode_block_raw(const Sched &s, uint32_t b, uint32_t &q, uint32_t &chunk);
__device__ __forceinline__ bool decode_block(const Sched &s, uint32_t b, uint32_t &q, uint32_t &chunk) {
	if (!decode_block_raw(s, b, q, chunk)) return false;
	return s.mode == 3 || q >= 64u || !((s.skip >> q) & 1ull);
}
__device__ __forceinline__ bool decode_block_raw(const Sched &s, uint32_t b, uint32_t &q, uint32_t &chunk) {
	if (s.mode == 3) {
// ... 559 lines not shown
__device__ __forceinline__ bool resolve_block(const ForestDev &fo, const Lvl &L, const int (&k)[3], const uint32_t (&p)[3],
                                              uint32_t (&pl)[3], uint32_t &owner) {
	int kk[3];
	bool changed = false;
#pragma unroll
	for (int d = 0; d < 3; ++d) {
		if (p[d] == 0u) { kk[d] = k[d] - 1; pl[d] = L.res[d] - 1u; changed = true; }
		else if (p[d] == L.res[d] + 1u) { kk[d] = k[d] + 1; pl[d] = 0u; changed = true; }
		else { kk[d] = k[d]; pl[d] = p[d] - 1u; }
	}
	if (changed) {
		if (!fo.continuity) return false;
		const int32_t pidx = identify(fo, (int16_t)kk[0], (int16_t)kk[1], (int16_t)kk[2]);
		const int32_t bi = pidx < 0 ? -1 : pidx - (int32_t)fo.level_poffset;
		if (bi < 0) return false;
		owner = (uint32_t)bi;
	}
	return true;
}

__device__ __forceinline__ bool resolve(const ForestDev &fo, const Batch &ba, const Lvl &L, const Block &b,
                                        const uint32_t (&p)[3], uint32_t (&pl)[3], uint32_t &offset) {
	uint32_t owner = 0xFFFFFFFFu;
	if (!resolve_block(fo, L, b.k, p, pl, owner)) return false;
	offset = (owner == 0xFFFFFFFFu) ? b.offset : (ba.offsets ? (uint32_t)ba.offsets[owner] : owner * ba.n_params);
	return true;
}

__device__ __forceinline__ void locate_forest(const float (&xp)[3], const Lvl &L, bool smooth, Cell<3> &c) {
#pragma unroll
	for (int d = 0; d < 3; ++d) {
		const float sc = (float)L.res[d];
		const float v = __fmaf_rn(xp[d], sc, 0.5f);
		const float fl = floorf(v);
		const float t = v - fl;
		c.sc[d] = sc;
		c.g[d] = (uint32_t)fl;
		if (!smooth) {
			c.w[d] = t; c.dw[d] = 1.0f; c.ddw[d] = 0.0f;
		} else {
			c.w[d] = t * t * __fmaf_rn(-2.0f, t, 3.0f);
			c.dw[d] = 6.0f * t * (1.0f - t);
			c.ddw[d] = __fmaf_rn(-12.0f, t, 6.0f);
		}
	}
}

uint64_t dparam_workspace_bytes(const nr3d_lotd_meta_t *m, uint32_t n_points, uint32_t n_batches, bool forest = false);
void set_dparam_chunk_log2(int lg);
int dparam_binned(bool second, const nr3d_lotd_meta_t *meta, const void *meta_dev, uint32_t N, const float *dL_ddLdx,
                  const float *dL_dy, int64_t g_sn, int64_t g_se, const float *x, const float *params, const Batch &batch,
                  uint32_t n_batches, int32_t max_level, float *dparam, void *workspace, uint64_t workspace_bytes,
                  hipStream_t st, bool &handled, const ForestDev *forest = nullptr, int32_t min_level = 0, bool g_half = false,
                  bool out_half = false, bool assign = false, bool p_half = false);

bool pair_applies(const nr3d_lotd_meta_t *m);
uint32_t pair_direct_levels(const nr3d_lotd_meta_t *m, uint32_t n_points);
void pair_layout(const nr3d_lotd_meta_t *m, uint32_t n_chunk, uint32_t units, uint64_t &rec_bytes, uint64_t &offs_bytes,
                 uint64_t &plan_bytes, uint64_t &part_bytes);
int pair_chunk(const nr3d_lotd_meta_t *meta, const nr3d_lotd_meta_t *md, uint32_t n, const float *x, const float *g,
               int64_t g_sn, int64_t g_se, int32_t min_level, int32_t max_level, uint32_t units, float *dparam,
               uint32_t out_flags , void *rec, uint32_t *offs, uint32_t *plan_buf, float *partial, hipStream_t st,
               const float *vin = nullptr );

}
}
```

nr3d_lib_amd/csrc/lotd_pair.hip:

```cpp
#include "lotd_device.h"
#include <stdlib.h>


namespace nr3d {
namespace lotd {

constexpr uint32_t kPEpbMax = 8192;
constexpr int kPAccThreads = 1024;
constexpr int kPLdsMax = 2 * (int)kPEpbMax;
constexpr int kPMaxLv = 32;
constexpr uint32_t kPMaxNb = 511;
typedef uint32_t u32x4 __attribute__((ext_vector_type(4)));

struct PairPlan {
	uint32_t qmap[kPMaxLv];
	uint32_t nb[kPMaxLv];
	uint32_t epb[kPMaxLv];
	uint32_t shift[kPMaxLv];
	uint32_t bucket_base[kPMaxLv + 1];
	uint32_t offs_base[kPMaxLv];
	uint32_t n_blk, n_pseudo;
	uint32_t cap;
	uint32_t lg;
	uint32_t sum_log2;
// ... 302 lines not shown
	const uint32_t i = blk * kPBP + threadIdx.x;
	for (uint32_t b = threadIdx.x; b <= nb; b += kPBP) hist[b] = 0;
	__syncthreads();
	const bool active = (i < n) && ((int32_t)level <= max_level);
	float xp[3] = {0.0f, 0.0f, 0.0f}, vin[3] = {0.0f, 0.0f, 0.0f}, g0 = 0.0f, g1 = 0.0f;
	if (active) {
#pragma unroll
		for (int d = 0; d < 3; ++d) xp[d] = x[(size_t)i * 3 + d];
		g0 = g[(int64_t)i * g_sn + (int64_t)(q * 2) * g_se];
		g1 = g[(int64_t)i * g_sn + (int64_t)(q * 2 + 1) * g_se];
		if constexpr (SECOND) {
#pragma unroll
			for (int d = 0; d < 3; ++d) vin[d] = vin_[(size_t)i * 3 + d];
		}
	}
	pair_level<kPBP, SECOND>(plan, ql, L, active, xp, g0, g1, smooth, stage, hist, nullptr, scan_lds,
	                         rec + ((size_t)ql * plan.n_blk + blk) * (size_t)plan.cap, offs_g + plan.offs_base[ql] + blk, plan.n_blk, vin,
	                         quad_on != 0u);
	if (gmax) {
		uint32_t gbits;
		if constexpr (!SECOND) {
			gbits = max(__float_as_uint(g0) & 0x7FFFFFFFu, __float_as_uint(g1) & 0x7FFFFFFFu);
			if (ql == 0 && i < n)
				for (uint32_t e = 0; e < dp.n; ++e) {
					const uint32_t qd = dp.qmap[e];
					if ((int32_t)meta_level_of(md, qd) > max_level) continue;
					gbits = max(gbits, __float_as_uint(g[(int64_t)i * g_sn + (int64_t)(qd * 2) * g_se]) & 0x7FFFFFFFu);
					gbits = max(gbits, __float_as_uint(g[(int64_t)i * g_sn + (int64_t)(qd * 2 + 1) * g_se]) & 0x7FFFFFFFu);
				}
		} else {
			auto bound = [&](const Lvl &Lq, float ga, float gb) {
				const float m = fmaxf(fabsf(ga), fabsf(gb)) * 1.5f *
				                ((float)(Lq.res[0] - 2u) * fabsf(vin[0]) + (float)(Lq.res[1] - 2u) * fabsf(vin[1]) + (float)(Lq.res[2] - 2u) * fabsf(vin[2]));
				return __float_as_uint(m) & 0x7FFFFFFFu;
			};
			gbits = bound(L, g0, g1);
			if (ql == 0 && i < n) {
				if (!active) {
#pragma unroll
					for (int d = 0; d < 3; ++d) vin[d] = vin_[(size_t)i * 3 + d];
				}
				for (uint32_t e = 0; e < dp.n; ++e) {
					const uint32_t qd = dp.qmap[e];
					if ((int32_t)meta_level_of(md, qd) > max_level) continue;
					const Lvl Ld = load_level(md, meta_level_of(md, qd));
					gbits = max(gbits, bound(Ld, g[(int64_t)i * g_sn + (int64_t)(qd * 2) * g_se], g[(int64_t)i * g_sn + (int64_t)(qd * 2 + 1) * g_se]));
				}
			}
		}
		pair_gmax<kPBP>(gbits, scan_lds, gmax);
	}
}

__global__ __launch_bounds__(1024) void k_pair_plan(PairPlan plan, const uint32_t *__restrict__ offs_g, uint32_t n_units,
                                                    uint32_t *__restrict__ tot, uint32_t *__restrict__ rep,
                                                    uint32_t *__restrict__ item_start, uint32_t *__restrict__ ticket) {
	__shared__ uint64_t red[16];
	__shared__ uint64_t carry_s;
	__shared__ uint32_t last_s;
	const uint32_t lane = threadIdx.x & 63, wave = threadIdx.x >> 6;
	const uint32_t NB = plan.bucket_base[plan.n_pseudo];
	{
		const uint32_t fb = blockIdx.x * 16 + wave;
		if (fb < NB) {
			uint32_t q = 0;
			while (q + 1 < plan.n_pseudo && plan.bucket_base[q + 1] <= fb) ++q;
			const uint32_t *ob0 = offs_g + plan.offs_base[q] + (size_t)(fb - plan.bucket_base[q]) * plan.n_blk;
			const uint32_t *ob1 = ob0 + plan.n_blk;
			uint32_t sum = 0;
			for (uint32_t blk = lane; blk < plan.n_blk; blk += 64) sum += ob1[blk] - ob0[blk];
#pragma unroll
			for (int off = 32; off >= 1; off >>= 1) sum += __shfl_xor(sum, off, 64);
			if (lane == 0) __hip_atomic_store(tot + fb, sum, __ATOMIC_RELAXED, __HIP_MEMORY_SCOPE_AGENT);
		}
	}
	__syncthreads();
	if (threadIdx.x == 0) {
		__builtin_amdgcn_fence(__ATOMIC_RELEASE, "agent");
		asm volatile("s_waitcnt vmcnt(0)" ::: "memory");
		last_s = (atomicAdd(ticket, 1u) == gridDim.x - 1u) ? 1u : 0u;
		__builtin_amdgcn_fence(__ATOMIC_ACQUIRE, "agent");
	}
	__syncthreads();
	if (!last_s) return;
	auto ld_tot = [&](uint32_t fb) { return (uint64_t)__hip_atomic_load(tot + fb, __ATOMIC_RELAXED, __HIP_MEMORY_SCOPE_AGENT); };
	uint64_t part = 0;
	for (uint32_t fb = threadIdx.x; fb < NB; fb += 1024) part += ld_tot(fb);
#pragma unroll
	for (int off = 32; off >= 1; off >>= 1) part += __shfl_xor(part, off, 64);
	if (lane == 0) red[wave] = part;
	__syncthreads();
	uint64_t total = 0;
#pragma unroll
	for (int w = 0; w < 16; ++w) total += red[w];
	const uint64_t unit = total / n_units > 0 ? total / n_units : 1;
	if (threadIdx.x == 0) carry_s = 0;
	__syncthreads();
	for (uint32_t base = 0; base < NB; base += 1024) {
		const uint32_t fb = base + threadIdx.x;
		uint32_t r = 0;
		if (fb < NB) {
			const uint64_t t = ld_tot(fb);
			r = t == 0 ? 0u : (uint32_t)((t + unit / 2) / unit);
			if (t != 0 && r < 1) r = 1;
			if (r > plan.n_blk) r = plan.n_blk;
			rep[fb] = r;
		}
		uint64_t inc = r;
#pragma unroll
		for (int off = 1; off < 64; off <<= 1) { const uint64_t t2 = __shfl_up(inc, off, 64); if ((int)lane >= off) inc += t2; }
		__syncthreads();
		if (lane == 63) red[wave] = inc;
		__syncthreads();
		uint64_t woff = 0, tsum = 0;
#pragma unroll
		for (int w = 0; w < 16; ++w) { if (w < (int)wave) woff += red[w]; tsum += red[w]; }
		const uint64_t c = carry_s;
		if (fb < NB) item_start[fb] = (uint32_t)(c + woff + inc - r);
		__syncthreads();
		if (threadIdx.x == 0) carry_s = c + tsum;
		__syncthreads();
	}
	if (threadIdx.x == 0) item_start[NB] = (uint32_t)carry_s;
}

__device__ __forceinline__ float *pair_target(const Lvl &L, uint32_t epb, uint32_t lg, uint32_t foff0, uint32_t b, uint32_t t,
                                              float *__restrict__ dparam, bool out_half = false) {
	const uint32_t f = t >> lg, el = t & ((1u << lg) - 1u);
	const uint64_t entry = (uint64_t)b * epb + el;
	if (el >= epb || entry >= L.size) return nullptr;
	const uint64_t at = L.off + (entry * L.F + foff0 + f);
	return out_half ? reinterpret_cast<float *>(reinterpret_cast<__half *>(dparam) + at) : dparam + at;
}
__device__ __forceinline__ float pair_ld(const float *p, bool out_half) {
	return out_half ? __half2float(*reinterpret_cast<const __half *>(p)) : *p;
}
__device__ __forceinline__ void pair_st(float *p, float v, bool out_half) {
	if (out_half) *reinterpret_cast<__half *>(p) = __float2half(v); else *p = v;
}

struct PairFix { double scale, inv; bool on; };
__device__ __forceinline__ PairFix pair_fix(const uint32_t *__restrict__ gmax, uint32_t sum_log2) {
	PairFix f;
	const uint32_t bits = ((cu32_t)gmax)[0];
	f.on = bits < 0x7F800000u;
	const int e = max((int)(bits >> 23), 1) - 126;
	const int lim = min(62 - (int)sum_log2, 50 - 6);
	const int sc = max(min(lim - e, 1000), -1000);
	f.scale = __longlong_as_double((long long)(sc + 1023) << 52);
	f.inv = __longlong_as_double((long long)(1023 - sc) << 52);
	return f;
}
__device__ __forceinline__ unsigned long long to_fix(float v, double scale) {
	const double t = __fma_rn((double)v, scale, 0x1.8p52);
	return (unsigned long long)(__double_as_longlong(t) - 0x4338000000000000LL);
}

template <int kUnroll, bool FIX>
__global__ __launch_bounds__(kPAccThreads, 8)  void k_pair_accum(PairPlan plan, const nr3d_lotd_meta_t *__restrict__ md,
                                                             const u32x4 *__restrict__ rec,
                                                             const uint32_t *__restrict__ offs_g,
                                                             const uint32_t *__restrict__ rep_g,
                                                             const uint32_t *__restrict__ item_start,
                                                             const uint32_t *__restrict__ gmax,
                                                             float *__restrict__ partial, float *__restrict__ dparam NR3D_DBG_PARAM,
                                                             uint32_t out_half) {
	NR3D_DBG_DECL
	extern __shared__ __attribute__((aligned(16))) unsigned long long acc_raw[];
	double *acc = reinterpret_cast<double *>(acc_raw);
	const uint32_t NB = plan.bucket_base[plan.n_pseudo];
	const cu32_t istart = (cu32_t)item_start, irep = (cu32_t)rep_g;
	if (blockIdx.x >= istart[NB]) return;
	uint32_t lo = 0, hi = NB;
	while (hi - lo > 1) { const uint32_t mid = (lo + hi) >> 1; if (istart[mid] <= blockIdx.x) lo = mid; else hi = mid; }
	const uint32_t fb = lo, R = irep[fb], r = blockIdx.x - istart[fb];
	uint32_t q = 0;
	while (q + 1 < plan.n_pseudo && plan.bucket_base[q + 1] <= fb) ++q;
	const uint32_t b = fb - plan.bucket_base[q];
	const uint32_t qg = plan.qmap[q];
	const Lvl L = load_level(md, meta_level_of(md, qg));
	const uint32_t foff0 = meta_cnt_of(md, qg) * 2u, epb = plan.epb[q];
	PairFix fx = {1.0, 1.0, false};
	if constexpr (FIX) fx = pair_fix(gmax, plan.sum_log2);
	const bool fix = FIX && fx.on;

	const uint32_t kPEpb = 1u << plan.lg, kPLds = 2u << plan.lg;
	for (uint32_t t = threadIdx.x; t < kPLds; t += kPAccThreads) acc_raw[t] = 0ull;
	__syncthreads();

	const uint32_t lane = threadIdx.x & 63, wave = threadIdx.x >> 6;
	constexpr uint32_t n_waves = kPAccThreads / 64;
	const uint32_t blk_lo = 0u, blk_hi = (plan.n_blk > r) ? (plan.n_blk - r + R - 1u) / R : 0u;
	const uint32_t *ob0 = offs_g + plan.offs_base[q] + (size_t)b * plan.n_blk;
	const uint32_t *ob1 = ob0 + plan.n_blk;
	const uint32_t kPCap = plan.cap;
	const u32x4 *rec_q = rec + (size_t)q * plan.n_blk * (size_t)kPCap;
	const uint32_t per_wave = (blk_hi - blk_lo + n_waves - 1) / n_waves;
	const uint32_t w_lo = min(blk_lo + wave * per_wave, blk_hi), w_hi = min(w_lo + per_wave, blk_hi);
	constexpr int kGroup = 8;
	for (uint32_t blk0 = w_lo; blk0 < w_hi; blk0 += 64) {
		const uint32_t mb = blk0 + lane;
		const uint32_t s_l = (mb < w_hi) ? ob0[r + R * mb] : 0u;
		const uint32_t e_l = (mb < w_hi) ? ob1[r + R * mb] : 0u;
		const uint32_t n_run = min(64u, w_hi - blk0);
		const u32x4 *rec_b = rec_q + (size_t)(r + R * blk0) * kPCap;
		for (uint32_t j0 = 0; j0 < n_run; j0 += kGroup) {
			uint32_t pre[kGroup + 1], rbase[kGroup];
			pre[0] = 0;
#pragma unroll
			for (int u = 0; u < kGroup; ++u) {
				const uint32_t j = min(j0 + (uint32_t)u, 63u);
				const uint32_t s_j = __builtin_amdgcn_readlane(s_l, j), e_j = __builtin_amdgcn_readlane(e_l, j);
				const uint32_t nrec = (j0 + (uint32_t)u < n_run) ? e_j - s_j : 0u;
				rbase[u] = s_j + j * R * kPCap - pre[u];
				pre[u + 1] = pre[u] + nrec;
			}
			const uint32_t total = pre[kGroup];
			for (uint32_t p0 = 0; p0 < total; p0 += 64u * kUnroll) {
				u32x4 rv[kUnroll];
#pragma unroll
				for (int v = 0; v < kUnroll; ++v) {
					const uint32_t pos = p0 + 64u * (uint32_t)v + lane;
					uint32_t at = rbase[0];
#pragma unroll
					for (int u = 1; u < kGroup; ++u) at = (pos >= pre[u]) ? rbase[u] : at;
					rv[v] = __builtin_nontemporal_load(rec_b + (size_t)((pos < total && !(dbg & 2u)) ? at + pos : rbase[0]));
				}
#pragma unroll
				for (int v = 0; v < kUnroll; ++v)
					if (p0 + 64u * (uint32_t)v + lane < total && !(dbg & 1u)) {
						const uint32_t h = rv[v].x, fl = (h >> 26) & 7u;
						const uint32_t i0 = h & 8191u, i1 = (h >> 13) & 8191u;
						const float w = __uint_as_float(rv[v].y), a0 = __uint_as_float(rv[v].z), a1 = __uint_as_float(rv[v].w);
						if (fl == 4u) {
							const uint32_t wyq = (((h >> 13) & 8191u) << 8) | (rv[v].y >> 24) | ((h >> 29) << 21), wzq = rv[v].y & 0xFFFFFFu;
							const float wy = (float)wyq * (1.0f / 16777215.0f), wz = (float)wzq * (1.0f / 16777215.0f);
							const float q00 = (1.0f - wy) * (1.0f - wz), q01 = (1.0f - wy) * wz, q10 = wy * (1.0f - wz), q11 = wy * wz;
							const uint32_t i2 = i0 + L.res[2];
							if (fix) {
								atomicAdd(&acc_raw[i0], to_fix(q00 * a0, fx.scale)); atomicAdd(&acc_raw[kPEpb + i0], to_fix(q00 * a1, fx.scale));
								atomicAdd(&acc_raw[i0 + 1u], to_fix(q01 * a0, fx.scale)); atomicAdd(&acc_raw[kPEpb + i0 + 1u], to_fix(q01 * a1, fx.scale));
								atomicAdd(&acc_raw[i2], to_fix(q10 * a0, fx.scale)); atomicAdd(&acc_raw[kPEpb + i2], to_fix(q10 * a1, fx.scale));
								atomicAdd(&acc_raw[i2 + 1u], to_fix(q11 * a0, fx.scale)); atomicAdd(&acc_raw[kPEpb + i2 + 1u], to_fix(q11 * a1, fx.scale));
							} else {
								atomicAdd(&acc[i0], (double)(q00 * a0)); atomicAdd(&acc[kPEpb + i0], (double)(q00 * a1));
								atomicAdd(&acc[i0 + 1u], (double)(q01 * a0)); atomicAdd(&acc[kPEpb + i0 + 1u], (double)(q01 * a1));
								atomicAdd(&acc[i2], (double)(q10 * a0)); atomicAdd(&acc[kPEpb + i2], (double)(q10 * a1));
								atomicAdd(&acc[i2 + 1u], (double)(q11 * a0)); atomicAdd(&acc[kPEpb + i2 + 1u], (double)(q11 * a1));
							}
							continue;
						}
						const bool pair = fl == 3u;
						const float wl = pair ? 1.0f - w : 1.0f, wh = pair ? w : 1.0f;
						if (fix) {
							if (fl & 1u) { atomicAdd(&acc_raw[i0], to_fix(wl * a0, fx.scale)); atomicAdd(&acc_raw[kPEpb + i0], to_fix(wl * a1, fx.scale)); }
							if (fl & 2u) { atomicAdd(&acc_raw[i1], to_fix(wh * a0, fx.scale)); atomicAdd(&acc_raw[kPEpb + i1], to_fix(wh * a1, fx.scale)); }
						} else {
							if (fl & 1u) { atomicAdd(&acc[i0], (double)(wl * a0)); atomicAdd(&acc[kPEpb + i0], (double)(wl * a1)); }
							if (fl & 2u) { atomicAdd(&acc[i1], (double)(wh * a0)); atomicAdd(&acc[kPEpb + i1], (double)(wh * a1)); }
						}
					}
			}
		}
	}
	__syncthreads();

	auto value = [&](uint32_t t) -> float {
		return fix ? (float)((double)(long long)acc_raw[t] * fx.inv) : (float)acc[t];
	};
	if (R > 1) {
		float *mine = partial + (size_t)blockIdx.x * kPLds;
		for (uint32_t t = threadIdx.x; t < kPLds; t += kPAccThreads) mine[t] = value(t);
		return;
	}
	constexpr int kFlush = 8;
	for (uint32_t tb = threadIdx.x; tb < kPLds; tb += kPAccThreads * kFlush) {
		float *p[kFlush];
		float v[kFlush], old[kFlush];
#pragma unroll
		for (int k = 0; k < kFlush; ++k) {
			const uint32_t t = tb + (uint32_t)k * kPAccThreads;
			p[k] = (t < kPLds) ? pair_target(L, epb, plan.lg, foff0, b, t, dparam, (out_half & 1u) != 0) : nullptr;
			v[k] = p[k] ? value(t) : 0.0f;
		}
		const bool half_out = (out_half & 1u) != 0, assign = (out_half & 2u) != 0;
#pragma unroll
		for (int k = 0; k < kFlush; ++k) old[k] = (p[k] && !assign) ? pair_ld(p[k], half_out) : 0.0f;
#pragma unroll
		for (int k = 0; k < kFlush; ++k) if (p[k]) pair_st(p[k], old[k] + v[k], half_out);
	}
}

template <bool FIX, bool SECOND = false>
__global__ __launch_bounds__(kPAccThreads, 8) void k_pair_direct(DirectPlan dp, const nr3d_lotd_meta_t *__restrict__ md, uint32_t n,
                                                                 int32_t max_level, uint32_t smooth, const float *__restrict__ x,
                                                                 const float *__restrict__ g, int64_t g_sn, int64_t g_se,
                                                                 const uint32_t *__restrict__ gmax, float *__restrict__ partial,
                                                                 const float *__restrict__ vin_) {
	extern __shared__ __attribute__((aligned(16))) unsigned long long acc_raw[];
	__shared__ uint32_t queue[kPAccThreads / 64][128];
	double *acc = reinterpret_cast<double *>(acc_raw);
	const uint32_t r = blockIdx.x, fb = blockIdx.y;
	uint32_t e = 0;
	while (e + 1 < dp.n && dp.bucket_base[e + 1] <= fb) ++e;
	const uint32_t b = fb - dp.bucket_base[e], q = dp.qmap[e];
	const uint32_t level = meta_level_of(md, q);
	const Lvl L = load_level(md, level);
	const uint32_t kPEpb = 1u << dp.lg, kPLds = 2u << dp.lg;
	PairFix fx = {1.0, 1.0, false};
	if constexpr (FIX) fx = pair_fix(gmax, dp.sum_log2);
	const bool fix = FIX && fx.on;
	for (uint32_t t = threadIdx.x; t < kPLds; t += kPAccThreads) acc_raw[t] = 0ull;
	__syncthreads();
	if ((int32_t)level <= max_level) {
		const uint32_t p_lo = r * dp.pts_per_rep;
		auto process = [&](uint32_t i) {
			float xp[3];
#pragma unroll
			for (int d = 0; d < 3; ++d) xp[d] = x[(size_t)i * 3 + d];
			const float g0 = g[(int64_t)i * g_sn + (int64_t)(q * 2) * g_se], g1 = g[(int64_t)i * g_sn + (int64_t)(q * 2 + 1) * g_se];
			uint32_t hdr[4], bkt[4], cell[3];
			constexpr int kW = SECOND ? 3 : 0;
			float A[4][2], wp[SECOND ? 4 : 1], vin[3] = {0.0f, 0.0f, 0.0f};
			bool valid;
			if constexpr (SECOND) {
#pragma unroll
				for (int d = 0; d < 3; ++d) vin[d] = vin_[(size_t)i * 3 + d];
			}
			uint32_t qmask;
			float wy_unused;
			pair_records<SECOND>(L, dp.shift[e], dp.epb[e], dp.lg, xp, g0, g1, smooth != 0, hdr, bkt, A, wp, cell, dp.nb[e], valid, vin, qmask, wy_unused, false);
			float lo[4][2], hi[4][2];
#pragma unroll
			for (int m = 0; m < 4; ++m)
#pragma unroll
				for (int f = 0; f < 2; ++f) { lo[m][f] = (1.0f - wp[m & kW]) * A[m][f]; hi[m][f] = wp[m & kW] * A[m][f]; }
			bool rotate = false;
			{
				const uint32_t ln = threadIdx.x & 63u;
				auto prev = [](uint32_t v) { return (uint32_t)__builtin_amdgcn_update_dpp(0, (int)v, 0x138, 0xf, 0xf, false); };
				bool same = ln > 0;
#pragma unroll
				for (int d = 0; d < 3; ++d) same = same && (prev(cell[d]) == cell[d]);
				same = same && (prev(1u) != 0u);
				rotate = (uint32_t)__popcll(__ballot(same)) >= dp.merge_min;
			}
			if (!valid) return;
			if (rotate) {
				const uint32_t ln = threadIdx.x & 63u;
				const bool sw = (ln & 4u) != 0u, fs = (ln & 8u) != 0u;
#pragma unroll
				for (uint32_t step = 0; step < 4u; ++step) {
					const uint32_t m = (step + ln) & 3u;
					auto sel = [&](auto a0, auto a1, auto a2, auto a3) { return m == 0u ? a0 : (m == 1u ? a1 : (m == 2u ? a2 : a3)); };
					if (sel(bkt[0], bkt[1], bkt[2], bkt[3]) != b) continue;
					const uint32_t hd = sel(hdr[0], hdr[1], hdr[2], hdr[3]);
					const float l0 = sel(lo[0][0], lo[1][0], lo[2][0], lo[3][0]), l1 = sel(lo[0][1], lo[1][1], lo[2][1], lo[3][1]);
					const float h0 = sel(hi[0][0], hi[1][0], hi[2][0], hi[3][0]), h1 = sel(hi[0][1], hi[1][1], hi[2][1], hi[3][1]);
					const uint32_t i0 = hd & 8191u, i1 = (hd >> 13) & 8191u;
					const uint32_t ea = sw ? i1 : i0, eb = sw ? i0 : i1;
					const float a0 = sw ? h0 : l0, a1 = sw ? h1 : l1, b0 = sw ? l0 : h0, b1 = sw ? l1 : h1;
					const uint32_t fa = fs ? kPEpb : 0u, fb2 = fs ? 0u : kPEpb;
					if (fix) {
// ... 49 lines not shown
					__builtin_amdgcn_wave_barrier();
					if (lane < rest) qw[lane] = t;
					qn = rest;
					__builtin_amdgcn_wave_barrier();
				}
			}
			if (lane < qn) process(qw[lane]);
		}
	}
	__syncthreads();
	float *mine = partial + ((size_t)fb * dp.R + r) * kPLds;
	for (uint32_t t = threadIdx.x; t < kPLds; t += kPAccThreads)
		mine[t] = fix ? (float)((double)(long long)acc_raw[t] * fx.inv) : (float)acc[t];
}

__global__ __launch_bounds__(kPAccThreads) void k_pair_direct_reduce(DirectPlan dp, const nr3d_lotd_meta_t *__restrict__ md,
                                                                     const float *__restrict__ partial, float *__restrict__ dparam,
                                                                     uint32_t out_half) {
	const uint32_t fb = blockIdx.x;
	const bool half_out = (out_half & 1u) != 0, assign = (out_half & 2u) != 0;
	uint32_t e = 0;
	while (e + 1 < dp.n && dp.bucket_base[e + 1] <= fb) ++e;
	const uint32_t b = fb - dp.bucket_base[e], q = dp.qmap[e];
	const Lvl L = load_level(md, meta_level_of(md, q));
	const uint32_t foff0 = meta_cnt_of(md, q) * 2u, kPLds = 2u << dp.lg;
	const uint32_t t = blockIdx.y * kPAccThreads + threadIdx.x;
	if (t >= kPLds) return;
	float *p = pair_target(L, dp.epb[e], dp.lg, foff0, b, t, dparam, half_out);
	if (!p) return;
	const float *part0 = partial + (size_t)fb * dp.R * kPLds + t;
	float sum = 0.0f;
	uint32_t r0 = 0;
	for (; r0 + 8 <= dp.R; r0 += 8) {
		float v[8];
#pragma unroll
		for (int j = 0; j < 8; ++j) v[j] = part0[(size_t)(r0 + j) * kPLds];
#pragma unroll
		for (int j = 0; j < 8; ++j) sum += v[j];
	}
	for (; r0 < dp.R; ++r0) sum += part0[(size_t)r0 * kPLds];
	pair_st(p, (assign ? 0.0f : pair_ld(p, half_out)) + sum, half_out);
}

constexpr uint32_t kRedRows = 4;
__global__ __launch_bounds__(kPAccThreads) void k_pair_reduce(PairPlan plan, const nr3d_lotd_meta_t *__restrict__ md,
                                                              const uint32_t *__restrict__ rep_g,
                                                              const uint32_t *__restrict__ item_start,
                                                              const float *__restrict__ partial, float *__restrict__ dparam,
                                                              uint32_t out_half, uint32_t NB, DirectPlan dp,
                                                              const float *__restrict__ dpart) {
	const bool half_out = (out_half & 1u) != 0, assign = (out_half & 2u) != 0;
	if (blockIdx.x >= NB) {
		const uint32_t fb = (blockIdx.x - NB) / kRedRows, sub = (blockIdx.x - NB) % kRedRows;
		uint32_t e = 0;
		while (e + 1 < dp.n && dp.bucket_base[e + 1] <= fb) ++e;
		const uint32_t b = fb - dp.bucket_base[e], q = dp.qmap[e];
		const Lvl L = load_level(md, meta_level_of(md, q));
		const uint32_t foff0 = meta_cnt_of(md, q) * 2u, kPLds = 2u << dp.lg;
		const uint32_t t = (blockIdx.y * kRedRows + sub) * kPAccThreads + threadIdx.x;
		if (t >= kPLds) return;
		float *p = pair_target(L, dp.epb[e], dp.lg, foff0, b, t, dparam, half_out);
		if (!p) return;
		const float *part0 = dpart + (size_t)fb * dp.R * kPLds + t;
		float sum = 0.0f;
		uint32_t r0 = 0;
		for (; r0 + 8 <= dp.R; r0 += 8) {
			float v[8];
#pragma unroll
			for (int j = 0; j < 8; ++j) v[j] = part0[(size_t)(r0 + j) * kPLds];
#pragma unroll
			for (int j = 0; j < 8; ++j) sum += v[j];
		}
		for (; r0 < dp.R; ++r0) sum += part0[(size_t)r0 * kPLds];
		pair_st(p, (assign ? 0.0f : pair_ld(p, half_out)) + sum, half_out);
		return;
	}
	const uint32_t fb = blockIdx.x;
	const uint32_t R = rep_g[fb];
	if (R == 1 || (R == 0 && !assign)) return;
	uint32_t q = 0;
	while (q + 1 < plan.n_pseudo && plan.bucket_base[q + 1] <= fb) ++q;
	const uint32_t b = fb - plan.bucket_base[q], qg = plan.qmap[q];
	const Lvl L = load_level(md, meta_level_of(md, qg));
	const uint32_t foff0 = meta_cnt_of(md, qg) * 2u;
	const uint32_t kPLds = 2u << plan.lg;
	const float *part0 = partial + (size_t)item_start[fb] * kPLds;
	for (uint32_t row = 0; row < kRedRows; ++row) {
		const uint32_t t = (blockIdx.y * kRedRows + row) * kPAccThreads + threadIdx.x;
		if (t >= kPLds) return;
		float *p = pair_target(L, plan.epb[q], plan.lg, foff0, b, t, dparam, half_out);
		if (!p) continue;
		float sum = 0.0f;
		uint32_t r0 = 0;
		for (; r0 + 8 <= R; r0 += 8) {
			float v[8];
#pragma unroll
			for (int j = 0; j < 8; ++j) v[j] = part0[(size_t)(r0 + j) * kPLds + t];
#pragma unroll
			for (int j = 0; j < 8; ++j) sum += v[j];
		}
		for (; r0 < R; ++r0) sum += part0[(size_t)r0 * kPLds + t];
		pair_st(p, (assign ? 0.0f : pair_ld(p, half_out)) + sum, half_out);
	}
}

static bool pair_enabled() { return opt::on(NR3D_OPT_LOTD_PAIR); }

bool pair_applies(const nr3d_lotd_meta_t *m) {
	if (!pair_enabled()) return false;
	if (!m || m->n_dims_to_encode != 3 || m->n_feat_per_pseudo_lvl != 2 || !m->c_hash_only) return false;
	if (m->n_pseudo_levels > (uint32_t)kPMaxLv) return false;
	for (uint32_t l = 0; l < m->n_levels; ++l) {
		const nr3d_lotd_level_t &L = m->levels[l];
		const uint32_t kPEpb = 1u << pair_lg();
		if (L.type == NR3D_LOD_Dense) {
			if (L.res[2] > kPEpb) return false;
			const uint64_t rows = (uint64_t)L.res[0] * L.res[1];
			uint32_t lg = 0;
			while ((2ull << lg) * L.res[2] <= kPEpb) ++lg;
			if (((rows + (1ull << lg) - 1) >> lg) > kPMaxNb) return false;
		} else if (L.type == NR3D_LOD_Hash) {
			if (L.size <= kPEpb) continue;
			if ((L.size & (L.size - 1u)) != 0u || L.res[0] > kPEpb) return false;
			if ((L.size >> pair_lg()) > kPMaxNb) return false;
		} else {
			return false;
		}
	}
	return true;
}


static void pair_plan(const nr3d_lotd_meta_t *m, uint32_t n_chunk, int32_t min_level, int32_t max_level, PairPlan &plan,
                      uint64_t &offs_words, uint64_t skip_pseudo = 0) {
	plan.n_blk = div_up(n_chunk, pair_bp());
	plan.cap = pair_bp() * 4u;
	plan.lg = pair_lg();
	plan.sum_log2 = 3;
	while ((1ull << (plan.sum_log2 - 3)) < n_chunk) ++plan.sum_log2;
	const uint32_t kPEpb = 1u << plan.lg;
	uint32_t nq = 0;
	uint64_t base = 0;
	for (uint32_t q = 0; q < m->n_pseudo_levels; ++q) {
		const int32_t lv = (int32_t)m->map_levels[q];
		if (lv < min_level || lv > max_level || ((skip_pseudo >> q) & 1ull)) continue;
		const nr3d_lotd_level_t &L = m->levels[lv];
		uint32_t nb, epb, sh;
		if (L.type == NR3D_LOD_Dense) {
			sh = 0;
			while ((2ull << sh) * L.res[2] <= kPEpb) ++sh;
			epb = (1u << sh) * L.res[2];
			nb = (uint32_t)((((uint64_t)L.res[0] * L.res[1]) + (1ull << sh) - 1) >> sh);
		} else {
			sh = plan.lg; epb = kPEpb;
// ... 12 lines not shown

static bool pair_direct_enabled() { return opt::on(NR3D_OPT_PAIR_DIRECT); }
static uint64_t pair_direct_plan(const PairPlan &full, uint32_t n, DirectPlan &dp) {
	dp.n = 0; dp.lg = full.lg; dp.sum_log2 = full.sum_log2; dp.R = 1; dp.pts_per_rep = n;
	dp.merge_min = (uint32_t)NR3D_XOPT(PAIR_DIRECT_ROTATE, 8);
	dp.bucket_base[0] = 0;
	if (!pair_direct_enabled()) return 0;
	uint64_t mask = 0;
	const int64_t nb_x = NR3D_XOPT(PAIR_DIRECT_NB, kDirectNb);
	const uint32_t nb_lim = nb_x < 0 ? 0u : (uint32_t)nb_x;
	for (uint32_t ql = 0; ql < full.n_pseudo && dp.n < kDirectMaxLv; ++ql) {
		if (full.nb[ql] > nb_lim || full.qmap[ql] >= 64u) continue;
		if (dp.bucket_base[dp.n] + full.nb[ql] > kDirectMaxWg) break;
		const uint32_t e = dp.n++;
		dp.qmap[e] = full.qmap[ql]; dp.nb[e] = full.nb[ql]; dp.epb[e] = full.epb[ql]; dp.shift[e] = full.shift[ql];
		dp.bucket_base[e + 1] = dp.bucket_base[e] + full.nb[ql];
		mask |= 1ull << full.qmap[ql];
	}
	if (dp.n == 0 || dp.n == full.n_pseudo) { dp.n = 0; return 0; }
	const uint32_t nbk = dp.bucket_base[dp.n];
	uint32_t R = kDirectMaxWg / nbk;
	R = R > 128u ? 128u : R;
	const uint32_t by_points = div_up(n, 2048u);
	R = R > by_points ? by_points : R;
	dp.R = R < 1u ? 1u : R;
	dp.pts_per_rep = div_up(n, dp.R);
	return mask;
}

uint32_t pair_direct_levels(const nr3d_lotd_meta_t *m, uint32_t n_points) {
	PairPlan plan;
	uint64_t ow;
	pair_plan(m, n_points, 0, 0x7fffffff, plan, ow);
	DirectPlan dp;
	pair_direct_plan(plan, n_points, dp);
	return dp.n;
}

void pair_layout(const nr3d_lotd_meta_t *m, uint32_t n_chunk, uint32_t units, uint64_t &rec_bytes, uint64_t &offs_bytes,
                 uint64_t &plan_bytes, uint64_t &part_bytes) {
	PairPlan plan;
	uint64_t ow;
	pair_plan(m, n_chunk, 0, 0x7fffffff, plan, ow);
	const uint32_t NB = plan.bucket_base[plan.n_pseudo];
	rec_bytes = (uint64_t)plan.n_pseudo * plan.n_blk * plan.cap * 16;
	offs_bytes = ((ow * 4 + 255) / 256) * 256;
	plan_bytes = (((uint64_t)NB * 3 + 4) * 4 + 255) / 256 * 256;
	part_bytes = (uint64_t)(pair_units() + NB + kDirectMaxWg) * (2u << plan.lg) * 4;
}

void launch_plan_items(uint32_t NB, uint32_t n_blk, uint32_t units, const uint32_t *tot, uint32_t *rep, uint32_t *item_start,
                       hipStream_t st);

int pair_chunk(const nr3d_lotd_meta_t *meta, const nr3d_lotd_meta_t *md, uint32_t n, const float *x, const float *g,
               int64_t g_sn, int64_t g_se, int32_t min_level, int32_t max_level, uint32_t units, float *dparam, uint32_t out_flags,
               void *rec, uint32_t *offs, uint32_t *plan_buf, float *partial, hipStream_t st, const float *vin) {
	PairPlan pl;
	uint64_t ow;
	pair_plan(meta, n, min_level, max_level, pl, ow);
	if (pl.n_pseudo == 0) return 0;
	DirectPlan dp;
	dp.n = 0;
	const uint32_t NB_full = pl.bucket_base[pl.n_pseudo];
	{
		const uint64_t skip = pair_direct_plan(pl, n, dp);
		if (skip) pair_plan(meta, n, min_level, max_level, pl, ow, skip);
	}
	uint32_t nb_max = 0;
	for (uint32_t q = 0; q < pl.n_pseudo; ++q) nb_max = nb_max > pl.nb[q] ? nb_max : pl.nb[q];
	const uint32_t NB = pl.bucket_base[pl.n_pseudo];
	uint32_t *tot = plan_buf, *rep = plan_buf + NB, *item_start = plan_buf + 2 * (size_t)NB;
	uint32_t *gmax = plan_buf + 3 * (size_t)NB + 2;
	units = pair_units();
	const size_t bin_lds_max = (size_t)1024 * 4 * 16 + (size_t)(kPMaxNb + 2) * 8;
	static bool attr_set_dev[64] = {};
	int dev_id = 0;
	NR3D_HIP_CHECK(hipGetDevice(&dev_id));
	if (!attr_set_dev[dev_id & 63]) {
#ifdef NR3D_EXPERIMENTS
		NR3D_HIP_CHECK(hipFuncSetAttribute((const void *)k_pair_bin<512>, hipFuncAttributeMaxDynamicSharedMemorySize, (int)bin_lds_max));
		NR3D_HIP_CHECK(hipFuncSetAttribute((const void *)k_pair_bin<768>, hipFuncAttributeMaxDynamicSharedMemorySize, (int)bin_lds_max));
		NR3D_HIP_CHECK(hipFuncSetAttribute((const void *)k_pair_bin<512, true>, hipFuncAttributeMaxDynamicSharedMemorySize, (int)bin_lds_max));
		NR3D_HIP_CHECK(hipFuncSetAttribute((const void *)k_pair_bin<768, true>, hipFuncAttributeMaxDynamicSharedMemorySize, (int)bin_lds_max));
		NR3D_HIP_CHECK(hipFuncSetAttribute((const void *)k_pair_accum<8, false>, hipFuncAttributeMaxDynamicSharedMemorySize, kPLdsMax * 8));
		NR3D_HIP_CHECK(hipFuncSetAttribute((const void *)k_pair_accum<8, true>, hipFuncAttributeMaxDynamicSharedMemorySize, kPLdsMax * 8));
#endif
		NR3D_HIP_CHECK(hipFuncSetAttribute((const void *)k_pair_bin<1024>, hipFuncAttributeMaxDynamicSharedMemorySize, (int)bin_lds_max));
		NR3D_HIP_CHECK(hipFuncSetAttribute((const void *)k_pair_bin<1024, true>, hipFuncAttributeMaxDynamicSharedMemorySize, (int)bin_lds_max));
		NR3D_HIP_CHECK(hipFuncSetAttribute((const void *)k_pair_direct<true>, hipFuncAttributeMaxDynamicSharedMemorySize, kPLdsMax * 8));
		NR3D_HIP_CHECK(hipFuncSetAttribute((const void *)k_pair_direct<false>, hipFuncAttributeMaxDynamicSharedMemorySize, kPLdsMax * 8));
		NR3D_HIP_CHECK(hipFuncSetAttribute((const void *)k_pair_direct<true, true>, hipFuncAttributeMaxDynamicSharedMemorySize, kPLdsMax * 8));
		NR3D_HIP_CHECK(hipFuncSetAttribute((const void *)k_pair_direct<false, true>, hipFuncAttributeMaxDynamicSharedMemorySize, kPLdsMax * 8));
		NR3D_HIP_CHECK(hipFuncSetAttribute((const void *)k_pair_accum<4, false>, hipFuncAttributeMaxDynamicSharedMemorySize, kPLdsMax * 8));
		NR3D_HIP_CHECK(hipFuncSetAttribute((const void *)k_pair_accum<4, true>, hipFuncAttributeMaxDynamicSharedMemorySize, kPLdsMax * 8));
		attr_set_dev[dev_id & 63] = true;
	}
	NR3D_HIP_CHECK(hipMemsetAsync(gmax, 0, 2 * sizeof(uint32_t), st));
	const uint32_t bp = pair_bp();
	const size_t bin_lds = (size_t)bp * 4 * 16 + (size_t)(nb_max + 1) * 4;
	const uint32_t quad_on = (!vin && pair_quad_enabled()) ? 1u : 0u;
#define NR3D_PAIR_BIN(BP) if (vin) NR3D_PAIR_BIN_(BP, true); else NR3D_PAIR_BIN_(BP, false)
#define NR3D_PAIR_BIN_(BP, SEC) hipLaunchKernelGGL((k_pair_bin<BP, SEC>), dim3(pl.n_blk, pl.n_pseudo), dim3(BP), bin_lds, st, pl, md, n, max_level, \
	meta->interpolation_type, x, g, g_sn, g_se, (u32x4 *)rec, offs, gmax, dp, vin, quad_on)
	{
		prof::Scope ps(NR3D_PROF_LOTD_BIN, st);
#ifdef NR3D_EXPERIMENTS
		if (bp == 512) { NR3D_PAIR_BIN(512); } else if (bp == 768) { NR3D_PAIR_BIN(768); } else
#endif
		{ NR3D_PAIR_BIN(1024); }
	}
#undef NR3D_PAIR_BIN
#undef NR3D_PAIR_BIN_
	float *dpart = partial + (size_t)(units + NB_full) * (2u << pl.lg);
	const uint32_t nbk_direct = dp.n ? dp.bucket_base[dp.n] : 0u;
	if (dp.n) {
		prof::Scope ps(NR3D_PROF_LOTD_DIRECT, st);
		auto direct = [&](auto kern) {
			hipLaunchKernelGGL(kern, dim3(dp.R, nbk_direct), dim3(kPAccThreads), (size_t)(16u << pl.lg), st, dp, md, n, max_level,
			                   meta->interpolation_type, x, g, g_sn, g_se, gmax, dpart, vin);
		};
		if (vin) { if (pair_fixed()) direct(k_pair_direct<true, true>); else direct(k_pair_direct<false, true>); }
		else     { if (pair_fixed()) direct(k_pair_direct<true, false>); else direct(k_pair_direct<false, false>); }
	}
	if (pl.n_pseudo == 0) {
		if (dp.n)
			hipLaunchKernelGGL(k_pair_direct_reduce, dim3(nbk_direct, (2u << pl.lg) / kPAccThreads), dim3(kPAccThreads), 0, st, dp, md, dpart,
			                   dparam, out_flags);
		NR3D_LAUNCH_CHECK();
		return 0;
	}
	hipLaunchKernelGGL(k_pair_plan, dim3(div_up(NB, 16)), dim3(1024), 0, st, pl, offs, units, tot, rep, item_start, gmax + 1);
#define NR3D_PAIR_ACC(U, F) hipLaunchKernelGGL((k_pair_accum<U, F>), dim3(units + NB), dim3(kPAccThreads), (size_t)(16u << pl.lg), st, pl, md, \
	(const u32x4 *)rec, offs, rep, item_start, gmax, partial, dparam NR3D_DBG_ARG(NR3D_XOPT(PAIR_DEBUG, 0)), out_flags)
	{
		prof::Scope ps(NR3D_PROF_LOTD_ACCUM, st);
#ifdef NR3D_EXPERIMENTS
		if (pair_unroll() == 8) { if (pair_fixed()) NR3D_PAIR_ACC(8, true); else NR3D_PAIR_ACC(8, false); } else
#endif
		{ if (pair_fixed()) NR3D_PAIR_ACC(4, true); else NR3D_PAIR_ACC(4, false); }
	}
#undef NR3D_PAIR_ACC
	hipLaunchKernelGGL(k_pair_reduce, dim3(NB + nbk_direct * kRedRows, div_up((2u << pl.lg) / kPAccThreads, kRedRows)), dim3(kPAccThreads), 0, st, pl, md, rep,
	                   item_start, partial, dparam, out_flags, NB, dp, dpart);
	NR3D_LAUNCH_CHECK();
	return 0;
}

}
}
```

Baseline: 1110 Mpoints/s.

## Fold gradient-max, plan and reduce stages of pair dparam into neighbouring kernels

Adds a 'pair fold' hand-over buffer. The dx contraction kernel computes the per-block max of |dL_dy|, which was previously found during binning, and zeroes the ticket/head area. The plan kernel is folded into extra rows of the direct kernel, and the final reduce is folded into the accumulate kernel through per-bucket tickets. This removes a memset, a separate plan launch and the reduce launch, plus some redundant scans. In exchange it adds cross-kernel coupling, ticket-based completion logic and extra work in the contract kernel.

```diff
diff --git a/include/nr3d_hip.h b/include/nr3d_hip.h
--- a/include/nr3d_hip.h
+++ b/include/nr3d_hip.h
@@ -8,7 +8,7 @@
 
 enum { NR3D_F32 = 0, NR3D_F16 = 1, NR3D_F64 = 2, NR3D_I32 = 3, NR3D_I64 = 4, NR3D_U8 = 5, NR3D_I16 = 6, NR3D_I8 = 7 };
 
-#define NR3D_ABI_VERSION 11
+#define NR3D_ABI_VERSION 12
 
 const char *nr3d_last_error(void);
 int nr3d_abi_version(void);
@@ -51,7 +51,8 @@
 	NR3D_OPT_DIRECT_FIXED = 19,
 	NR3D_OPT_VM_SORTED = 20,
 	NR3D_OPT_MLP_X3 = 21,
-	NR3D_OPT_COUNT = 22
+	NR3D_OPT_PAIR_FOLD = 22,
+	NR3D_OPT_COUNT = 23
 };
 int nr3d_set_option(int id, int64_t value);
 int64_t nr3d_get_option(int id);
@@ -132,6 +133,14 @@
                                const void *dL_dy, int64_t g_sn, int64_t g_se, const void *x, int32_t max_level,
                                int out_dtype, int assign, void *dL_dparam, void *workspace, uint64_t workspace_bytes,
                                void *stream);
+uint64_t nr3d_lotd_pair_fold_bytes(const nr3d_lotd_meta_t *meta, uint32_t n_points, int32_t max_level);
+int nr3d_lotd_bwd_dx_fold(const nr3d_lotd_meta_t *meta, uint32_t n_points, int x_dtype, int param_dtype, const void *dL_dy,
+                          int64_t dldy_sn, int64_t dldy_se, const void *dy_dx, int64_t dydx_sn, int64_t dydx_se, void *dL_dx,
+                          void *dL_dy_T, int32_t max_level, void *fold, void *stream);
+int nr3d_lotd_bwd_dparam_typed_fold(const nr3d_lotd_meta_t *meta, const void *meta_dev, uint32_t n_points, int grad_dtype,
+                                    const void *dL_dy, int64_t g_sn, int64_t g_se, const void *x, int32_t max_level,
+                                    int out_dtype, int assign, void *dL_dparam, void *workspace, uint64_t workspace_bytes,
+                                    void *fold, void *stream);
 
 int nr3d_lotd_bwd_bwd_ddLdy(const nr3d_lotd_meta_t *meta, uint32_t n_points, int x_dtype, int param_dtype,
                             const void *dL_ddLdx, const void *dy_dx, int64_t dydx_sn, int64_t dydx_se,
diff --git a/nr3d_lib_amd/_abi.py b/nr3d_lib_amd/_abi.py
--- a/nr3d_lib_amd/_abi.py
+++ b/nr3d_lib_amd/_abi.py
@@ -1,4 +1,4 @@
-ABI_VERSION = 11
+ABI_VERSION = 12
 SIGNATURES = {
     'nr3d_abi_version': ('int', []),
     'nr3d_alpha_to_vw_backward': ('int', ['uint32_t', 'uint64_t', 'ptr', 'ptr', 'ptr', 'ptr', 'float', 'float', 'ptr', 'ptr']),
@@ -18,7 +18,9 @@
     'nr3d_lotd_bwd_dparam': ('int', ['ptr', 'ptr', 'uint32_t', 'int', 'int', 'ptr', 'int64_t', 'int64_t', 'ptr', 'ptr', 'ptr', 'ptr', 'uint32_t', 'uint32_t', 'int32_t', 'ptr', 'ptr', 'uint64_t', 'ptr']),
     'nr3d_lotd_bwd_dparam_levels': ('int', ['ptr', 'ptr', 'uint32_t', 'int', 'int', 'ptr', 'int64_t', 'int64_t', 'ptr', 'ptr', 'ptr', 'ptr', 'uint32_t', 'uint32_t', 'int32_t', 'int32_t', 'ptr', 'ptr', 'uint64_t', 'ptr']),
     'nr3d_lotd_bwd_dparam_typed': ('int', ['ptr', 'ptr', 'uint32_t', 'int', 'ptr', 'int64_t', 'int64_t', 'ptr', 'int32_t', 'int', 'int', 'ptr', 'ptr', 'uint64_t', 'ptr']),
+    'nr3d_lotd_bwd_dparam_typed_fold': ('int', ['ptr', 'ptr', 'uint32_t', 'int', 'ptr', 'int64_t', 'int64_t', 'ptr', 'int32_t', 'int', 'int', 'ptr', 'ptr', 'uint64_t', 'ptr', 'ptr']),
     'nr3d_lotd_bwd_dx': ('int', ['ptr', 'uint32_t', 'int', 'int', 'ptr', 'int64_t', 'int64_t', 'ptr', 'int64_t', 'int64_t', 'ptr', 'ptr', 'ptr']),
+    'nr3d_lotd_bwd_dx_fold': ('int', ['ptr', 'uint32_t', 'int', 'int', 'ptr', 'int64_t', 'int64_t', 'ptr', 'int64_t', 'int64_t', 'ptr', 'ptr', 'int32_t', 'ptr', 'ptr']),
     'nr3d_lotd_dLdy_feature_major': ('int', ['uint32_t', 'uint32_t', 'int', 'ptr', 'int64_t', 'int64_t', 'ptr', 'ptr']),
     'nr3d_lotd_dparam_workspace_bytes': ('uint64_t', ['ptr', 'uint32_t', 'uint32_t']),
     'nr3d_lotd_forest_bwd_bwd_dx': ('int', ['ptr', 'ptr', 'ptr', 'uint32_t', 'ptr', 'ptr', 'ptr', 'ptr', 'int', 'ptr', 'ptr', 'uint32_t', 'int32_t', 'ptr', 'ptr']),
@@ -34,6 +36,7 @@
     'nr3d_lotd_mlp_forward': ('int', ['ptr', 'ptr', 'uint64_t', 'ptr', 'ptr', 'int', 'int32_t', 'ptr', 'ptr', 'ptr', 'int64_t', 'uint32_t', 'ptr']),
     'nr3d_lotd_mlp_forward_ok': ('int', ['ptr', 'ptr']),
     'nr3d_lotd_pair_direct_levels': ('int', ['ptr', 'uint32_t']),
+    'nr3d_lotd_pair_fold_bytes': ('uint64_t', ['ptr', 'uint32_t', 'int32_t']),
     'nr3d_lotd_pair_path_ok': ('int', ['ptr']),
     'nr3d_lotd_set_dparam_chunk_log2': ('void', ['int']),
     'nr3d_march_composite_bwd': ('int', ['uint32_t', 'ptr', 'ptr', 'ptr', 'ptr', 'ptr', 'float', 'float', 'int', 'ptr', 'ptr', 'ptr', 'ptr', 'ptr', 'ptr', 'ptr', 'ptr', 'ptr', 'ptr', 'uint64_t', 'ptr', 'ptr']),
diff --git a/nr3d_lib_amd/_hip.py b/nr3d_lib_amd/_hip.py
--- a/nr3d_lib_amd/_hip.py
+++ b/nr3d_lib_amd/_hip.py
@@ -129,7 +129,8 @@
 
 OPTION_IDS = dict(lotd_pair=0, pair_quad=1, pair_second=2, pair_direct=3, pair_fixed=4, fwd_pairlane=5, fwd_split=6,
                   fwd_lds_stage=7, hvp_levels=8, hvp_pairlane=9, hvp_split=10, vm_split=11, cp_direct=12, march_group=13,
-                  pack_scan=14, vm_lines_direct=15, fwd_cell_major=16, sort_wave=17, vm_direct=18, direct_fixed=19, vm_sorted=20, mlp_x3=21)
+                  pack_scan=14, vm_lines_direct=15, fwd_cell_major=16, sort_wave=17, vm_direct=18, direct_fixed=19, vm_sorted=20, mlp_x3=21,
+                  pair_fold=22)
 
 
 def set_option(name, value):
diff --git a/nr3d_lib_amd/bindings/_lotd.py b/nr3d_lib_amd/bindings/_lotd.py
--- a/nr3d_lib_amd/bindings/_lotd.py
+++ b/nr3d_lib_amd/bindings/_lotd.py
@@ -421,23 +421,29 @@
         st = H.stream_of(input)
         tag = ("dx" if need_input_grad else "") + ("dp" if need_param_grad else "")
         with _Prof(m, f"LoTD{D}-bwd-{tag}", N):
-            gT = None
+            gT = fold = None
             if need_input_grad and N > 0:
                 j, jsn, jse = _jac_view(dy_dx.detach(), N, E, D)
                 if (need_param_grad and not batched and USE_BINNED_DPARAM and gse == 1 and gsn == E
                         and g32.data_ptr() % 16 == 0):
                     gT = H.empty((E, N), dtype=torch.float32, device=dev)
-                H.check(H.lib().nr3d_lotd_bwd_dx(
+                    if typed:
+                        fb = H.lib().nr3d_lotd_pair_fold_bytes
+                        fb.restype = C.c_uint64
+                        nfold = int(fb(C.byref(m._cmeta()), H.u32(N), H.i32(max_level)))
+                        if nfold:
+                            fold = H.empty(((nfold + 3) // 4,), dtype=torch.int32, device=dev)
+                H.check(H.lib().nr3d_lotd_bwd_dx_fold(
                     C.byref(m._cmeta()), H.u32(N), C.c_int(H.F32), C.c_int(gcode), H.ptr(g32), H.i64(gsn),
-                    H.i64(gse), H.ptr(j), H.i64(jsn), H.i64(jse), H.ptr(dL_dx), H.ptr(gT), st))
+                    H.i64(gse), H.ptr(j), H.i64(jsn), H.i64(jse), H.ptr(dL_dx), H.ptr(gT), H.i32(max_level), H.ptr(fold), st))
             if need_param_grad and N > 0 and typed:
                 ws, wsb = _dparam_workspace(m, N, dev, 1)
                 if gT is not None:
                     g32, gsn, gse, gcode = gT, 1, N, H.F32
-                H.check(H.lib().nr3d_lotd_bwd_dparam_typed(
+                H.check(H.lib().nr3d_lotd_bwd_dparam_typed_fold(
                     C.byref(m._cmeta()), H.ptr(m._dev(dev)), H.u32(N), C.c_int(gcode), H.ptr(g32), H.i64(gsn), H.i64(gse),
                     H.ptr(_f32c(input.detach())), H.i32(max_level), C.c_int(H.F16 if native else H.F32), C.c_int(1),
-                    H.ptr(dL_dparam), H.ptr(ws), C.c_uint64(wsb), st))
+                    H.ptr(dL_dparam), H.ptr(ws), C.c_uint64(wsb), H.ptr(fold), st))
             elif need_param_grad and N > 0:
                 x32, (p32, pcode) = _f32c(input.detach()), _ptab(params)
                 nbat = _n_batches(m, p32, batch_offsets, batched)
diff --git a/nr3d_lib_amd/csrc/host_api.hip b/nr3d_lib_amd/csrc/host_api.hip
--- a/nr3d_lib_amd/csrc/host_api.hip
+++ b/nr3d_lib_amd/csrc/host_api.hip
@@ -52,9 +52,9 @@
 	 1,  1,  1,  1,  1,  1,
 	 1,  1,  1,  1,  1,  1,
 	 1,  0,  1,  0,  1,  1,
-	 1,  1,  1,  1,
+	 1,  1,  1,  1,  1,
 };
-std::atomic<int64_t> g_val[NR3D_OPT_COUNT] = {1, 1, 1, 1, 1, 1, 1, 1, 1, 1, 1, 1, 1, 0, 1, 0, 1, 1, 1, 1, 1, 1};
+std::atomic<int64_t> g_val[NR3D_OPT_COUNT] = {1, 1, 1, 1, 1, 1, 1, 1, 1, 1, 1, 1, 1, 0, 1, 0, 1, 1, 1, 1, 1, 1, 1};
 
 #ifdef NR3D_EXPERIMENTS
 int64_t experiment_env(const char *name, int64_t dflt) {
diff --git a/nr3d_lib_amd/csrc/lotd.hip b/nr3d_lib_amd/csrc/lotd.hip
--- a/nr3d_lib_amd/csrc/lotd.hip
+++ b/nr3d_lib_amd/csrc/lotd.hip
@@ -1225,11 +1225,17 @@
 __global__ __launch_bounds__(kBlock) void k_contract_dx_rowmajor(uint32_t N, uint32_t E, const GT *__restrict__ dL_dy,
                                                                  const float *__restrict__ dydx, int64_t d_sn,
                                                                  int64_t d_se, float *__restrict__ dL_dx,
-                                                                 float *__restrict__ dL_dy_T) {
+                                                                 float *__restrict__ dL_dy_T, uint32_t *__restrict__ fold,
+                                                                 uint32_t gcols, uint32_t n_zero, uint32_t slot_off) {
 	constexpr int TE = 32;
 	__shared__ float tile[TE][kBlock + 1];
+	__shared__ uint32_t gred[kBlock / 64];
 	const uint32_t i0 = blockIdx.x * kBlock, i = i0 + threadIdx.x;
 	const uint32_t n_here = min((uint32_t)kBlock, N - i0);
+	uint32_t gbits = 0;
+	auto gm = [&](uint32_t e, float v) { if (e < gcols) gbits = max(gbits, __float_as_uint(v) & 0x7FFFFFFFu); };
+	if (fold && blockIdx.x == 0)
+		for (uint32_t k = threadIdx.x; k < n_zero; k += kBlock) fold[k] = 0u;
 	float acc[D];
 #pragma unroll
 	for (int d = 0; d < D; ++d) acc[d] = 0.0f;
@@ -1249,12 +1255,16 @@
 						t = make_float4(a.x, a.y, b.x, b.y);
 					}
 					tile[e4][p] = t.x; tile[e4 + 1][p] = t.y; tile[e4 + 2][p] = t.z; tile[e4 + 3][p] = t.w;
+					if (fold) { gm(e0 + e4, t.x); gm(e0 + e4 + 1, t.y); gm(e0 + e4 + 2, t.z); gm(e0 + e4 + 3, t.w); }
 				}
 			}
 		} else {
 			for (uint32_t v = threadIdx.x; v < kBlock * te; v += kBlock) {
 				const uint32_t p = v / te, e = v - p * te;
-				if (p < n_here) tile[e][p] = to_f32<GT>(dL_dy[(size_t)(i0 + p) * E + e0 + e]);
+				if (p < n_here) {
+					tile[e][p] = to_f32<GT>(dL_dy[(size_t)(i0 + p) * E + e0 + e]);
+					if (fold) gm(e0 + e, tile[e][p]);
+				}
 			}
 		}
 		__syncthreads();
@@ -1277,6 +1287,17 @@
 	if (i < N) {
 #pragma unroll
 		for (int d = 0; d < D; ++d) dL_dx[(size_t)i * D + d] = acc[d];
+	}
+	if (fold) {
+#pragma unroll
+		for (int off = 32; off >= 1; off >>= 1) gbits = max(gbits, (uint32_t)__shfl_xor((int)gbits, off, 64));
+		if ((threadIdx.x & 63u) == 0) gred[threadIdx.x >> 6] = gbits;
+		__syncthreads();
+		if (threadIdx.x == 0) {
+#pragma unroll
+			for (int k = 1; k < kBlock / 64; ++k) gbits = max(gbits, gred[k]);
+			fold[slot_off + blockIdx.x] = gbits;
+		}
 	}
 }
 
@@ -1701,9 +1722,9 @@
 	return 0;
 }
 
-extern "C" int nr3d_lotd_bwd_dx(const nr3d_lotd_meta_t *meta, uint32_t N, int x_dtype, int param_dtype,
-                                const void *dL_dy, int64_t g_sn, int64_t g_se, const void *dy_dx, int64_t d_sn,
-                                int64_t d_se, void *dL_dx, void *dL_dy_T, void *stream) {
+static int bwd_dx(const nr3d_lotd_meta_t *meta, uint32_t N, int x_dtype, int param_dtype, const void *dL_dy, int64_t g_sn,
+                  int64_t g_se, const void *dy_dx, int64_t d_sn, int64_t d_se, void *dL_dx, void *dL_dy_T, int32_t max_level,
+                  void *fold_buf, void *stream) {
 	NR3D_CHECK(meta != nullptr, "LoTD: meta is NULL");
 	NR3D_CHECK(x_dtype == NR3D_F32 && (param_dtype == NR3D_F32 || param_dtype == NR3D_F16), "LoTD::bwd_dx: f32 x, f32 / f16 dL_dy");
 	if (N == 0) return 0;
@@ -1713,20 +1734,42 @@
 	const bool row_major = (g_se == 1 && g_sn == (int64_t)E && ((uintptr_t)dL_dy % (g_half ? 8 : 16)) == 0);
 	NR3D_CHECK(dL_dy_T == nullptr || row_major, "LoTD::bwd_dx: dL_dy_T needs a contiguous, 16-byte aligned [N, E] dL_dy");
 	NR3D_CHECK(!g_half || (row_major && (E & 3u) == 0u), "LoTD::bwd_dx: half dL_dy must be a contiguous [N, E] tensor, E % 4 == 0");
+	uint32_t gcols = 0, n_zero = 0, slot_off = 0;
+	uint32_t *fold = (fold_buf && pair_fold_layout(meta, N, max_level, gcols, n_zero, slot_off) != 0) ? (uint32_t *)fold_buf : nullptr;
+	NR3D_CHECK(!fold || row_major, "LoTD::bwd_dx_fold: the hand-over buffer needs a contiguous, 16-byte aligned [N, E] dL_dy");
 	prof::Scope ps(NR3D_PROF_LOTD_CONTRACT_DX, (hipStream_t)stream);
 	DISPATCH_D(meta->n_dims_to_encode, {
 		if (row_major && g_half)
 			hipLaunchKernelGGL((k_contract_dx_rowmajor<D, __half>), dim3(div_up(N, kBlock)), dim3(kBlock), 0, (hipStream_t)stream, N, E,
-			                   (const __half *)dL_dy, (const float *)dy_dx, d_sn, d_se, (float *)dL_dx, (float *)dL_dy_T);
+			                   (const __half *)dL_dy, (const float *)dy_dx, d_sn, d_se, (float *)dL_dx, (float *)dL_dy_T, fold, gcols,
+			                   n_zero, slot_off);
 		else if (row_major)
 			hipLaunchKernelGGL((k_contract_dx_rowmajor<D, float>), dim3(div_up(N, kBlock)), dim3(kBlock), 0, (hipStream_t)stream, N, E,
-			                   (const float *)dL_dy, (const float *)dy_dx, d_sn, d_se, (float *)dL_dx, (float *)dL_dy_T);
+			                   (const float *)dL_dy, (const float *)dy_dx, d_sn, d_se, (float *)dL_dx, (float *)dL_dy_T, fold, gcols,
+			                   n_zero, slot_off);
 		else
 			hipLaunchKernelGGL(k_contract_dx<D>, dim3(div_up(N, kBlock)), dim3(kBlock), 0, (hipStream_t)stream, N, E,
 			                   (const float *)dL_dy, g_sn, g_se, (const float *)dy_dx, d_sn, d_se, (float *)dL_dx);
 	});
 	NR3D_LAUNCH_CHECK();
 	return 0;
+}
+
+extern "C" int nr3d_lotd_bwd_dx(const nr3d_lotd_meta_t *meta, uint32_t N, int x_dtype, int param_dtype,
+                                const void *dL_dy, int64_t g_sn, int64_t g_se, const void *dy_dx, int64_t d_sn,
+                                int64_t d_se, void *dL_dx, void *dL_dy_T, void *stream) {
+	return bwd_dx(meta, N, x_dtype, param_dtype, dL_dy, g_sn, g_se, dy_dx, d_sn, d_se, dL_dx, dL_dy_T, 0, nullptr, stream);
+}
+
+extern "C" uint64_t nr3d_lotd_pair_fold_bytes(const nr3d_lotd_meta_t *meta, uint32_t N, int32_t max_level) {
+	uint32_t gcols, n_zero, slot_off;
+	return meta ? pair_fold_layout(meta, N, max_level, gcols, n_zero, slot_off) : 0;
+}
+
+extern "C" int nr3d_lotd_bwd_dx_fold(const nr3d_lotd_meta_t *meta, uint32_t N, int x_dtype, int param_dtype, const void *dL_dy,
+                                     int64_t g_sn, int64_t g_se, const void *dy_dx, int64_t d_sn, int64_t d_se, void *dL_dx,
+                                     void *dL_dy_T, int32_t max_level, void *fold, void *stream) {
+	return bwd_dx(meta, N, x_dtype, param_dtype, dL_dy, g_sn, g_se, dy_dx, d_sn, d_se, dL_dx, dL_dy_T, max_level, fold, stream);
 }
 
 static int launch_bwd_dparam(bool second, const nr3d_lotd_meta_t *meta, const void *meta_dev, uint32_t N,
@@ -1793,10 +1836,9 @@
 	return (meta && pair_applies(meta)) ? (int)pair_direct_levels(meta, n_points) : 0;
 }
 
-extern "C" int nr3d_lotd_bwd_dparam_typed(const nr3d_lotd_meta_t *meta, const void *meta_dev, uint32_t N, int grad_dtype,
-                                          const void *dL_dy, int64_t g_sn, int64_t g_se, const void *x, int32_t max_level,
-                                          int out_dtype, int assign, void *dL_dparam, void *workspace, uint64_t workspace_bytes,
-                                          void *stream) {
+static int bwd_dparam_typed(const nr3d_lotd_meta_t *meta, const void *meta_dev, uint32_t N, int grad_dtype, const void *dL_dy,
+                            int64_t g_sn, int64_t g_se, const void *x, int32_t max_level, int out_dtype, int assign, void *dL_dparam,
+                            void *workspace, uint64_t workspace_bytes, void *fold, void *stream) {
 	if (int rc = check_common(meta, meta_dev, NR3D_F32, NR3D_F32)) return rc;
 	NR3D_CHECK((grad_dtype == NR3D_F32 || grad_dtype == NR3D_F16) && (out_dtype == NR3D_F32 || out_dtype == NR3D_F16),
 	           "LoTD::bwd_dparam_typed: f32 / f16 only");
@@ -1810,10 +1852,26 @@
 	const Batch bb{nullptr, nullptr, 0u, meta->n_params};
 	if (int rc = dparam_binned(false, meta, meta_dev, N, nullptr, (const float *)dL_dy, g_sn, g_se, (const float *)x, nullptr, bb,
 	                           1u, max_level, (float *)dL_dparam, workspace, workspace_bytes, (hipStream_t)stream, handled, nullptr,
-	                           0, grad_dtype == NR3D_F16, out_dtype == NR3D_F16, assign != 0))
+	                           0, grad_dtype == NR3D_F16, out_dtype == NR3D_F16, assign != 0, false, (uint32_t *)fold))
 		return rc;
 	NR3D_CHECK(handled, "LoTD::bwd_dparam_typed: the pair-record path does not apply to this meta / workspace");
 	return 0;
+}
+
+extern "C" int nr3d_lotd_bwd_dparam_typed(const nr3d_lotd_meta_t *meta, const void *meta_dev, uint32_t N, int grad_dtype,
+                                          const void *dL_dy, int64_t g_sn, int64_t g_se, const void *x, int32_t max_level,
+                                          int out_dtype, int assign, void *dL_dparam, void *workspace, uint64_t workspace_bytes,
+                                          void *stream) {
+	return bwd_dparam_typed(meta, meta_dev, N, grad_dtype, dL_dy, g_sn, g_se, x, max_level, out_dtype, assign, dL_dparam, workspace,
+	                        workspace_bytes, nullptr, stream);
+}
+
+extern "C" int nr3d_lotd_bwd_dparam_typed_fold(const nr3d_lotd_meta_t *meta, const void *meta_dev, uint32_t N, int grad_dtype,
+                                               const void *dL_dy, int64_t g_sn, int64_t g_se, const void *x, int32_t max_level,
+                                               int out_dtype, int assign, void *dL_dparam, void *workspace, uint64_t workspace_bytes,
+                                               void *fold, void *stream) {
+	return bwd_dparam_typed(meta, meta_dev, N, grad_dtype, dL_dy, g_sn, g_se, x, max_level, out_dtype, assign, dL_dparam, workspace,
+	                        workspace_bytes, fold, stream);
 }
 
 extern "C" int nr3d_lotd_bwd_dparam_levels(const nr3d_lotd_meta_t *meta, const void *meta_dev, uint32_t N, int x_dtype,
diff --git a/nr3d_lib_amd/csrc/lotd_bin.hip b/nr3d_lib_amd/csrc/lotd_bin.hip
--- a/nr3d_lib_amd/csrc/lotd_bin.hip
+++ b/nr3d_lib_amd/csrc/lotd_bin.hip
@@ -957,6 +957,7 @@
 	const uint32_t chunk = 1u << (g_chunk_log2 ? g_chunk_log2 : 22);
 	return n < chunk ? n : chunk;
 }
+bool dparam_one_pass(uint32_t n) { return chunk_points(n) >= n; }
 
 constexpr int kCpThreads = 1024;
 constexpr uint32_t kCpMaxItems = 32, kCpLdsBytes = 144 * 1024, kCpReplicas = 128, kCpMaxPairs = 4;
@@ -1577,7 +1578,7 @@
                   const float *dL_dy, int64_t g_sn, int64_t g_se, const float *x, const float *params, const Batch &batch,
                   uint32_t n_batches, int32_t max_level, float *dparam, void *workspace, uint64_t workspace_bytes,
                   hipStream_t st, bool &handled, const ForestDev *forest, int32_t min_level, bool g_half, bool out_half, bool assign,
-                  bool p_half) {
+                  bool p_half, uint32_t *fold) {
 	handled = false;
 	BinLayout lay;
 	const uint32_t nc = chunk_points(N);
@@ -1630,7 +1631,7 @@
 			need_gt();
 			if (int rc = pair_chunk(meta, md, n, xc, gc, sn, se, min_level, max_level, work_units(), dparam,
 			                        (out_half ? 1u : 0u) | (assign_now ? 2u : 0u), rec, offs, plan_buf, partial, st,
-			                        second ? vc : nullptr))
+			                        second ? vc : nullptr, (N <= nc && !second) ? fold : nullptr))
 				return rc;
 			continue;
 		}
diff --git a/nr3d_lib_amd/csrc/lotd_device.h b/nr3d_lib_amd/csrc/lotd_device.h
--- a/nr3d_lib_amd/csrc/lotd_device.h
+++ b/nr3d_lib_amd/csrc/lotd_device.h
@@ -635,7 +635,8 @@
                   const float *dL_dy, int64_t g_sn, int64_t g_se, const float *x, const float *params, const Batch &batch,
                   uint32_t n_batches, int32_t max_level, float *dparam, void *workspace, uint64_t workspace_bytes,
                   hipStream_t st, bool &handled, const ForestDev *forest = nullptr, int32_t min_level = 0, bool g_half = false,
-                  bool out_half = false, bool assign = false, bool p_half = false);
+                  bool out_half = false, bool assign = false, bool p_half = false, uint32_t *fold = nullptr);
+bool dparam_one_pass(uint32_t n_points);
 
 bool pair_applies(const nr3d_lotd_meta_t *m);
 uint32_t pair_direct_levels(const nr3d_lotd_meta_t *m, uint32_t n_points);
@@ -644,7 +645,10 @@
 int pair_chunk(const nr3d_lotd_meta_t *meta, const nr3d_lotd_meta_t *md, uint32_t n, const float *x, const float *g,
                int64_t g_sn, int64_t g_se, int32_t min_level, int32_t max_level, uint32_t units, float *dparam,
                uint32_t out_flags , void *rec, uint32_t *offs, uint32_t *plan_buf, float *partial, hipStream_t st,
-               const float *vin = nullptr );
-
-}
-}
+               const float *vin = nullptr ,
+               uint32_t *fold = nullptr );
+uint64_t pair_fold_layout(const nr3d_lotd_meta_t *m, uint32_t n, int32_t max_level, uint32_t &gcols, uint32_t &zero_words,
+                          uint32_t &slot_off);
+
+}
+}
diff --git a/nr3d_lib_amd/csrc/lotd_pair.hip b/nr3d_lib_amd/csrc/lotd_pair.hip
--- a/nr3d_lib_amd/csrc/lotd_pair.hip
+++ b/nr3d_lib_amd/csrc/lotd_pair.hip
@@ -378,16 +378,33 @@
 	}
 }
 
-__global__ __launch_bounds__(1024) void k_pair_plan(PairPlan plan, const uint32_t *__restrict__ offs_g, uint32_t n_units,
-                                                    uint32_t *__restrict__ tot, uint32_t *__restrict__ rep,
-                                                    uint32_t *__restrict__ item_start, uint32_t *__restrict__ ticket) {
+__device__ __forceinline__ uint32_t gmax_slots(const uint32_t *__restrict__ slots, uint32_t n_slots, uint32_t *red) {
+	uint32_t m = 0;
+	for (uint32_t k = threadIdx.x; k < n_slots; k += 1024u) m = max(m, slots[k]);
+#pragma unroll
+	for (int off = 32; off >= 1; off >>= 1) m = max(m, (uint32_t)__shfl_xor((int)m, off, 64));
+	__syncthreads();
+	if ((threadIdx.x & 63u) == 0) red[threadIdx.x >> 6] = m;
+	__syncthreads();
+	m = 0;
+#pragma unroll
+	for (int k = 0; k < 16; ++k) m = max(m, red[k]);
+	__syncthreads();
+	return m;
+}
+
+__device__ __forceinline__ void pair_plan_block(const PairPlan &plan, const uint32_t *__restrict__ offs_g, uint32_t n_units,
+                                                uint32_t *__restrict__ tot, uint32_t *__restrict__ rep,
+                                                uint32_t *__restrict__ item_start, uint32_t *__restrict__ ticket, uint32_t bid,
+                                                uint32_t nblk, const uint32_t *__restrict__ slots, uint32_t n_slots,
+                                                uint32_t *__restrict__ gmax_out, bool empty_one) {
 	__shared__ uint64_t red[16];
 	__shared__ uint64_t carry_s;
 	__shared__ uint32_t last_s;
 	const uint32_t lane = threadIdx.x & 63, wave = threadIdx.x >> 6;
 	const uint32_t NB = plan.bucket_base[plan.n_pseudo];
 	{
-		const uint32_t fb = blockIdx.x * 16 + wave;
+		const uint32_t fb = bid * 16 + wave;
 		if (fb < NB) {
 			uint32_t q = 0;
 			while (q + 1 < plan.n_pseudo && plan.bucket_base[q + 1] <= fb) ++q;
@@ -404,11 +421,15 @@
 	if (threadIdx.x == 0) {
 		__builtin_amdgcn_fence(__ATOMIC_RELEASE, "agent");
 		asm volatile("s_waitcnt vmcnt(0)" ::: "memory");
-		last_s = (atomicAdd(ticket, 1u) == gridDim.x - 1u) ? 1u : 0u;
+		last_s = (atomicAdd(ticket, 1u) == nblk - 1u) ? 1u : 0u;
 		__builtin_amdgcn_fence(__ATOMIC_ACQUIRE, "agent");
 	}
 	__syncthreads();
 	if (!last_s) return;
+	if (slots) {
+		const uint32_t gb = gmax_slots(slots, n_slots, reinterpret_cast<uint32_t *>(red));
+		if (threadIdx.x == 0) gmax_out[0] = gb;
+	}
 	auto ld_tot = [&](uint32_t fb) { return (uint64_t)__hip_atomic_load(tot + fb, __ATOMIC_RELAXED, __HIP_MEMORY_SCOPE_AGENT); };
 	uint64_t part = 0;
 	for (uint32_t fb = threadIdx.x; fb < NB; fb += 1024) part += ld_tot(fb);
@@ -427,7 +448,7 @@
 		uint32_t r = 0;
 		if (fb < NB) {
 			const uint64_t t = ld_tot(fb);
-			r = t == 0 ? 0u : (uint32_t)((t + unit / 2) / unit);
+			r = t == 0 ? (empty_one ? 1u : 0u) : (uint32_t)((t + unit / 2) / unit);
 			if (t != 0 && r < 1) r = 1;
 			if (r > plan.n_blk) r = plan.n_blk;
 			rep[fb] = r;
@@ -448,6 +469,13 @@
 		__syncthreads();
 	}
 	if (threadIdx.x == 0) item_start[NB] = (uint32_t)carry_s;
+}
+__global__ __launch_bounds__(1024) void k_pair_plan(PairPlan plan, const uint32_t *__restrict__ offs_g, uint32_t n_units,
+                                                    uint32_t *__restrict__ tot, uint32_t *__restrict__ rep,
+                                                    uint32_t *__restrict__ item_start, uint32_t *__restrict__ ticket,
+                                                    const uint32_t *__restrict__ slots, uint32_t n_slots, uint32_t *__restrict__ gmax_out,
+                                                    uint32_t empty_one) {
+	pair_plan_block(plan, offs_g, n_units, tot, rep, item_start, ticket, blockIdx.x, gridDim.x, slots, n_slots, gmax_out, empty_one != 0u);
 }
 
 __device__ __forceinline__ float *pair_target(const Lvl &L, uint32_t epb, uint32_t lg, uint32_t foff0, uint32_t b, uint32_t t,
@@ -466,9 +494,8 @@
 }
 
 struct PairFix { double scale, inv; bool on; };
-__device__ __forceinline__ PairFix pair_fix(const uint32_t *__restrict__ gmax, uint32_t sum_log2) {
+__device__ __forceinline__ PairFix pair_fix_bits(uint32_t bits, uint32_t sum_log2) {
 	PairFix f;
-	const uint32_t bits = ((cu32_t)gmax)[0];
 	f.on = bits < 0x7F800000u;
 	const int e = max((int)(bits >> 23), 1) - 126;
 	const int lim = min(62 - (int)sum_log2, 50 - 6);
@@ -477,9 +504,41 @@
 	f.inv = __longlong_as_double((long long)(1023 - sc) << 52);
 	return f;
 }
+__device__ __forceinline__ PairFix pair_fix(const uint32_t *__restrict__ gmax, uint32_t sum_log2) {
+	return pair_fix_bits(((cu32_t)gmax)[0], sum_log2);
+}
 __device__ __forceinline__ unsigned long long to_fix(float v, double scale) {
 	const double t = __fma_rn((double)v, scale, 0x1.8p52);
 	return (unsigned long long)(__double_as_longlong(t) - 0x4338000000000000LL);
+}
+
+__device__ __forceinline__ float pair_replica_sum(const float *__restrict__ part_t, uint32_t R, uint32_t kPLds) {
+	float sum = 0.0f;
+	uint32_t r0 = 0;
+	for (; r0 + 8 <= R; r0 += 8) {
+		float v[8];
+#pragma unroll
+		for (int j = 0; j < 8; ++j) v[j] = part_t[(size_t)(r0 + j) * kPLds];
+#pragma unroll
+		for (int j = 0; j < 8; ++j) sum += v[j];
+	}
+	for (; r0 < R; ++r0) sum += part_t[(size_t)r0 * kPLds];
+	return sum;
+}
+__device__ __forceinline__ void pair_direct_sum(const DirectPlan &dp, const nr3d_lotd_meta_t *__restrict__ md,
+                                                const float *__restrict__ dpart, float *__restrict__ dparam, uint32_t out_half,
+                                                uint32_t fb, uint32_t t) {
+	const bool half_out = (out_half & 1u) != 0, assign = (out_half & 2u) != 0;
+	uint32_t e = 0;
+	while (e + 1 < dp.n && dp.bucket_base[e + 1] <= fb) ++e;
+	const uint32_t b = fb - dp.bucket_base[e], q = dp.qmap[e];
+	const Lvl L = load_level(md, meta_level_of(md, q));
+	const uint32_t foff0 = meta_cnt_of(md, q) * 2u, kPLds = 2u << dp.lg;
+	if (t >= kPLds) return;
+	float *p = pair_target(L, dp.epb[e], dp.lg, foff0, b, t, dparam, half_out);
+	if (!p) return;
+	const float sum = pair_replica_sum(dpart + (size_t)fb * dp.R * kPLds + t, dp.R, kPLds);
+	pair_st(p, (assign ? 0.0f : pair_ld(p, half_out)) + sum, half_out);
 }
 
 template <int kUnroll, bool FIX>
@@ -490,16 +549,24 @@
                                                              const uint32_t *__restrict__ item_start,
                                                              const uint32_t *__restrict__ gmax,
                                                              float *__restrict__ partial, float *__restrict__ dparam NR3D_DBG_PARAM,
-                                                             uint32_t out_half) {
+                                                             uint32_t out_half, uint32_t *__restrict__ bticket, uint32_t n_dred,
+                                                             DirectPlan dp, const float *__restrict__ dpart) {
 	NR3D_DBG_DECL
 	extern __shared__ __attribute__((aligned(16))) unsigned long long acc_raw[];
+	__shared__ uint32_t last_s;
+	if (blockIdx.x < n_dred) {
+		const uint32_t rows = (2u << dp.lg) / kPAccThreads;
+		pair_direct_sum(dp, md, dpart, dparam, out_half, blockIdx.x / rows, (blockIdx.x % rows) * kPAccThreads + threadIdx.x);
+		return;
+	}
+	const uint32_t item = blockIdx.x - n_dred;
 	double *acc = reinterpret_cast<double *>(acc_raw);
 	const uint32_t NB = plan.bucket_base[plan.n_pseudo];
 	const cu32_t istart = (cu32_t)item_start, irep = (cu32_t)rep_g;
-	if (blockIdx.x >= istart[NB]) return;
+	if (item >= istart[NB]) return;
 	uint32_t lo = 0, hi = NB;
-	while (hi - lo > 1) { const uint32_t mid = (lo + hi) >> 1; if (istart[mid] <= blockIdx.x) lo = mid; else hi = mid; }
-	const uint32_t fb = lo, R = irep[fb], r = blockIdx.x - istart[fb];
+	while (hi - lo > 1) { const uint32_t mid = (lo + hi) >> 1; if (istart[mid] <= item) lo = mid; else hi = mid; }
+	const uint32_t fb = lo, R = irep[fb], r = item - istart[fb];
 	uint32_t q = 0;
 	while (q + 1 < plan.n_pseudo && plan.bucket_base[q + 1] <= fb) ++q;
 	const uint32_t b = fb - plan.bucket_base[q];
@@ -595,8 +662,28 @@
 		return fix ? (float)((double)(long long)acc_raw[t] * fx.inv) : (float)acc[t];
 	};
 	if (R > 1) {
-		float *mine = partial + (size_t)blockIdx.x * kPLds;
+		float *mine = partial + (size_t)item * kPLds;
 		for (uint32_t t = threadIdx.x; t < kPLds; t += kPAccThreads) mine[t] = value(t);
+		if (!bticket) return;
+		asm volatile("s_waitcnt vmcnt(0)" ::: "memory");
+		__syncthreads();
+		if (threadIdx.x == 0) {
+			__builtin_amdgcn_fence(__ATOMIC_RELEASE, "agent");
+			asm volatile("s_waitcnt vmcnt(0)" ::: "memory");
+			last_s = (atomicAdd(bticket + fb, 1u) == R - 1u) ? 1u : 0u;
+			__builtin_amdgcn_fence(__ATOMIC_ACQUIRE, "agent");
+			asm volatile("s_waitcnt vmcnt(0)" ::: "memory");
+		}
+		__syncthreads();
+		if (!last_s) return;
+		const bool half_out = (out_half & 1u) != 0, assign = (out_half & 2u) != 0;
+		const float *part0 = partial + (size_t)istart[fb] * kPLds;
+		for (uint32_t t = threadIdx.x; t < kPLds; t += kPAccThreads) {
+			float *p = pair_target(L, epb, plan.lg, foff0, b, t, dparam, half_out);
+			if (!p) continue;
+			const float sum = pair_replica_sum(part0 + t, R, kPLds);
+			pair_st(p, (assign ? 0.0f : pair_ld(p, half_out)) + sum, half_out);
+		}
 		return;
 	}
 	constexpr int kFlush = 8;
@@ -622,9 +709,19 @@
                                                                  int32_t max_level, uint32_t smooth, const float *__restrict__ x,
                                                                  const float *__restrict__ g, int64_t g_sn, int64_t g_se,
                                                                  const uint32_t *__restrict__ gmax, float *__restrict__ partial,
-                                                                 const float *__restrict__ vin_) {
+                                                                 const float *__restrict__ vin_, uint32_t plan_rows, PairPlan plan,
+                                                                 const uint32_t *__restrict__ offs_g, uint32_t n_units,
+                                                                 uint32_t *__restrict__ tot, uint32_t *__restrict__ rep,
+                                                                 uint32_t *__restrict__ item_start, uint32_t *__restrict__ ticket,
+                                                                 const uint32_t *__restrict__ slots, uint32_t n_slots,
+                                                                 uint32_t *__restrict__ gmax_out, uint32_t empty_one) {
 	extern __shared__ __attribute__((aligned(16))) unsigned long long acc_raw[];
 	__shared__ uint32_t queue[kPAccThreads / 64][128];
+	if (blockIdx.y >= gridDim.y - plan_rows) {
+		const uint32_t bid = (blockIdx.y - (gridDim.y - plan_rows)) * gridDim.x + blockIdx.x, nblk = (plan.bucket_base[plan.n_pseudo] + 15u) / 16u;
+		if (bid < nblk) pair_plan_block(plan, offs_g, n_units, tot, rep, item_start, ticket, bid, nblk, slots, n_slots, gmax_out, empty_one != 0u);
+		return;
+	}
 	double *acc = reinterpret_cast<double *>(acc_raw);
 	const uint32_t r = blockIdx.x, fb = blockIdx.y;
 	uint32_t e = 0;
@@ -634,7 +731,7 @@
 	const Lvl L = load_level(md, level);
 	const uint32_t kPEpb = 1u << dp.lg, kPLds = 2u << dp.lg;
 	PairFix fx = {1.0, 1.0, false};
-	if constexpr (FIX) fx = pair_fix(gmax, dp.sum_log2);
+	if constexpr (FIX) fx = slots ? pair_fix_bits(gmax_slots(slots, n_slots, &queue[0][0]), dp.sum_log2) : pair_fix(gmax, dp.sum_log2);
 	const bool fix = FIX && fx.on;
 	for (uint32_t t = threadIdx.x; t < kPLds; t += kPAccThreads) acc_raw[t] = 0ull;
 	__syncthreads();
@@ -790,27 +887,7 @@
 	const bool half_out = (out_half & 1u) != 0, assign = (out_half & 2u) != 0;
 	if (blockIdx.x >= NB) {
 		const uint32_t fb = (blockIdx.x - NB) / kRedRows, sub = (blockIdx.x - NB) % kRedRows;
-		uint32_t e = 0;
-		while (e + 1 < dp.n && dp.bucket_base[e + 1] <= fb) ++e;
-		const uint32_t b = fb - dp.bucket_base[e], q = dp.qmap[e];
-		const Lvl L = load_level(md, meta_level_of(md, q));
-		const uint32_t foff0 = meta_cnt_of(md, q) * 2u, kPLds = 2u << dp.lg;
-		const uint32_t t = (blockIdx.y * kRedRows + sub) * kPAccThreads + threadIdx.x;
-		if (t >= kPLds) return;
-		float *p = pair_target(L, dp.epb[e], dp.lg, foff0, b, t, dparam, half_out);
-		if (!p) return;
-		const float *part0 = dpart + (size_t)fb * dp.R * kPLds + t;
-		float sum = 0.0f;
-		uint32_t r0 = 0;
-		for (; r0 + 8 <= dp.R; r0 += 8) {
-			float v[8];
-#pragma unroll
-			for (int j = 0; j < 8; ++j) v[j] = part0[(size_t)(r0 + j) * kPLds];
-#pragma unroll
-			for (int j = 0; j < 8; ++j) sum += v[j];
-		}
-		for (; r0 < dp.R; ++r0) sum += part0[(size_t)r0 * kPLds];
-		pair_st(p, (assign ? 0.0f : pair_ld(p, half_out)) + sum, half_out);
+		pair_direct_sum(dp, md, dpart, dparam, out_half, fb, (blockIdx.y * kRedRows + sub) * kPAccThreads + threadIdx.x);
 		return;
 	}
 	const uint32_t fb = blockIdx.x;
@@ -828,16 +905,7 @@
 		if (t >= kPLds) return;
 		float *p = pair_target(L, plan.epb[q], plan.lg, foff0, b, t, dparam, half_out);
 		if (!p) continue;
-		float sum = 0.0f;
-		uint32_t r0 = 0;
-		for (; r0 + 8 <= R; r0 += 8) {
-			float v[8];
-#pragma unroll
-			for (int j = 0; j < 8; ++j) v[j] = part0[(size_t)(r0 + j) * kPLds + t];
-#pragma unroll
-			for (int j = 0; j < 8; ++j) sum += v[j];
-		}
-		for (; r0 < R; ++r0) sum += part0[(size_t)r0 * kPLds + t];
+		const float sum = pair_replica_sum(part0 + t, R, kPLds);
 		pair_st(p, (assign ? 0.0f : pair_ld(p, half_out)) + sum, half_out);
 	}
 }
@@ -956,9 +1024,33 @@
 void launch_plan_items(uint32_t NB, uint32_t n_blk, uint32_t units, const uint32_t *tot, uint32_t *rep, uint32_t *item_start,
                        hipStream_t st);
 
+constexpr uint32_t kFoldHead = 64;
+uint64_t pair_fold_layout(const nr3d_lotd_meta_t *m, uint32_t n, int32_t max_level, uint32_t &gcols, uint32_t &zero_words,
+                          uint32_t &slot_off) {
+	gcols = zero_words = slot_off = 0;
+	if (!opt::on(NR3D_OPT_PAIR_FOLD) || !m || !pair_applies(m) || n == 0 || max_level < 0 || !dparam_one_pass(n)) return 0;
+	if (2u * m->n_pseudo_levels != m->n_encoded_dims) return 0;
+	uint32_t nq = 0;
+	while (nq < m->n_pseudo_levels && (int32_t)m->map_levels[nq] <= max_level) ++nq;
+	for (uint32_t q = nq; q < m->n_pseudo_levels; ++q)
+		if ((int32_t)m->map_levels[q] <= max_level) return 0;
+	if (nq == 0) return 0;
+	PairPlan pl;
+	uint64_t ow;
+	pair_plan(m, n, 0, max_level, pl, ow);
+	gcols = 2u * nq;
+	zero_words = kFoldHead + pl.bucket_base[pl.n_pseudo];
+	slot_off = (zero_words + 63u) & ~63u;
+	return (uint64_t)(slot_off + div_up(n, (uint32_t)kBlock)) * 4u;
+}
+
 int pair_chunk(const nr3d_lotd_meta_t *meta, const nr3d_lotd_meta_t *md, uint32_t n, const float *x, const float *g,
                int64_t g_sn, int64_t g_se, int32_t min_level, int32_t max_level, uint32_t units, float *dparam, uint32_t out_flags,
-               void *rec, uint32_t *offs, uint32_t *plan_buf, float *partial, hipStream_t st, const float *vin) {
+               void *rec, uint32_t *offs, uint32_t *plan_buf, float *partial, hipStream_t st, const float *vin, uint32_t *fold) {
+	uint32_t f_gcols = 0, f_zero = 0, f_slot = 0;
+	if (fold && (vin || min_level > 0 || pair_fold_layout(meta, n, max_level, f_gcols, f_zero, f_slot) == 0)) fold = nullptr;
+	const uint32_t *slots = fold ? fold + f_slot : nullptr;
+	const uint32_t n_slots = div_up(n, (uint32_t)kBlock);
 	PairPlan pl;
 	uint64_t ow;
 	pair_plan(meta, n, min_level, max_level, pl, ow);
@@ -974,7 +1066,8 @@
 	for (uint32_t q = 0; q < pl.n_pseudo; ++q) nb_max = nb_max > pl.nb[q] ? nb_max : pl.nb[q];
 	const uint32_t NB = pl.bucket_base[pl.n_pseudo];
 	uint32_t *tot = plan_buf, *rep = plan_buf + NB, *item_start = plan_buf + 2 * (size_t)NB;
-	uint32_t *gmax = plan_buf + 3 * (size_t)NB + 2;
+	uint32_t *gmax = fold ? fold : plan_buf + 3 * (size_t)NB + 2;
+	uint32_t *bticket = fold ? fold + kFoldHead : nullptr;
 	units = pair_units();
 	const size_t bin_lds_max = (size_t)1024 * 4 * 16 + (size_t)(kPMaxNb + 2) * 8;
 	static bool attr_set_dev[64] = {};
@@ -999,13 +1092,13 @@
 		NR3D_HIP_CHECK(hipFuncSetAttribute((const void *)k_pair_accum<4, true>, hipFuncAttributeMaxDynamicSharedMemorySize, kPLdsMax * 8));
 		attr_set_dev[dev_id & 63] = true;
 	}
-	NR3D_HIP_CHECK(hipMemsetAsync(gmax, 0, 2 * sizeof(uint32_t), st));
+	if (!fold) NR3D_HIP_CHECK(hipMemsetAsync(gmax, 0, 2 * sizeof(uint32_t), st));
 	const uint32_t bp = pair_bp();
 	const size_t bin_lds = (size_t)bp * 4 * 16 + (size_t)(nb_max + 1) * 4;
 	const uint32_t quad_on = (!vin && pair_quad_enabled()) ? 1u : 0u;
 #define NR3D_PAIR_BIN(BP) if (vin) NR3D_PAIR_BIN_(BP, true); else NR3D_PAIR_BIN_(BP, false)
 #define NR3D_PAIR_BIN_(BP, SEC) hipLaunchKernelGGL((k_pair_bin<BP, SEC>), dim3(pl.n_blk, pl.n_pseudo), dim3(BP), bin_lds, st, pl, md, n, max_level, \
-	meta->interpolation_type, x, g, g_sn, g_se, (u32x4 *)rec, offs, gmax, dp, vin, quad_on)
+	meta->interpolation_type, x, g, g_sn, g_se, (u32x4 *)rec, offs, fold ? nullptr : gmax, dp, vin, quad_on)
 	{
 		prof::Scope ps(NR3D_PROF_LOTD_BIN, st);
 #ifdef NR3D_EXPERIMENTS
@@ -1017,11 +1110,15 @@
 #undef NR3D_PAIR_BIN_
 	float *dpart = partial + (size_t)(units + NB_full) * (2u << pl.lg);
 	const uint32_t nbk_direct = dp.n ? dp.bucket_base[dp.n] : 0u;
+	const bool plan_in_direct = fold && dp.n && pl.n_pseudo;
+	const uint32_t plan_rows = plan_in_direct ? div_up(div_up(NB, 16u), dp.R) : 0u;
+	const uint32_t empty_one = (fold && (out_flags & 2u)) ? 1u : 0u;
 	if (dp.n) {
 		prof::Scope ps(NR3D_PROF_LOTD_DIRECT, st);
 		auto direct = [&](auto kern) {
-			hipLaunchKernelGGL(kern, dim3(dp.R, nbk_direct), dim3(kPAccThreads), (size_t)(16u << pl.lg), st, dp, md, n, max_level,
-			                   meta->interpolation_type, x, g, g_sn, g_se, gmax, dpart, vin);
+			hipLaunchKernelGGL(kern, dim3(dp.R, nbk_direct + plan_rows), dim3(kPAccThreads), (size_t)(16u << pl.lg), st, dp, md, n, max_level,
+			                   meta->interpolation_type, x, g, g_sn, g_se, gmax, dpart, vin, plan_rows, pl, offs, units, tot, rep, item_start,
+			                   gmax + 1, slots, n_slots, fold, empty_one);
 		};
 		if (vin) { if (pair_fixed()) direct(k_pair_direct<true, true>); else direct(k_pair_direct<false, true>); }
 		else     { if (pair_fixed()) direct(k_pair_direct<true, false>); else direct(k_pair_direct<false, false>); }
@@ -1033,9 +1130,12 @@
 		NR3D_LAUNCH_CHECK();
 		return 0;
 	}
-	hipLaunchKernelGGL(k_pair_plan, dim3(div_up(NB, 16)), dim3(1024), 0, st, pl, offs, units, tot, rep, item_start, gmax + 1);
-#define NR3D_PAIR_ACC(U, F) hipLaunchKernelGGL((k_pair_accum<U, F>), dim3(units + NB), dim3(kPAccThreads), (size_t)(16u << pl.lg), st, pl, md, \
-	(const u32x4 *)rec, offs, rep, item_start, gmax, partial, dparam NR3D_DBG_ARG(NR3D_XOPT(PAIR_DEBUG, 0)), out_flags)
+	if (!plan_in_direct)
+		hipLaunchKernelGGL(k_pair_plan, dim3(div_up(NB, 16)), dim3(1024), 0, st, pl, offs, units, tot, rep, item_start, gmax + 1, slots, n_slots,
+		                   fold, empty_one);
+	const uint32_t n_dred = fold ? nbk_direct * ((2u << pl.lg) / kPAccThreads) : 0u;
+#define NR3D_PAIR_ACC(U, F) hipLaunchKernelGGL((k_pair_accum<U, F>), dim3(n_dred + units + NB), dim3(kPAccThreads), (size_t)(16u << pl.lg), st, pl, md, \
+	(const u32x4 *)rec, offs, rep, item_start, gmax, partial, dparam NR3D_DBG_ARG(NR3D_XOPT(PAIR_DEBUG, 0)), out_flags, bticket, n_dred, dp, dpart)
 	{
 		prof::Scope ps(NR3D_PROF_LOTD_ACCUM, st);
 #ifdef NR3D_EXPERIMENTS
@@ -1044,8 +1144,9 @@
 		{ if (pair_fixed()) NR3D_PAIR_ACC(4, true); else NR3D_PAIR_ACC(4, false); }
 	}
 #undef NR3D_PAIR_ACC
-	hipLaunchKernelGGL(k_pair_reduce, dim3(NB + nbk_direct * kRedRows, div_up((2u << pl.lg) / kPAccThreads, kRedRows)), dim3(kPAccThreads), 0, st, pl, md, rep,
-	                   item_start, partial, dparam, out_flags, NB, dp, dpart);
+	if (!fold)
+		hipLaunchKernelGGL(k_pair_reduce, dim3(NB + nbk_direct * kRedRows, div_up((2u << pl.lg) / kPAccThreads, kRedRows)), dim3(kPAccThreads), 0, st, pl, md, rep,
+		                   item_start, partial, dparam, out_flags, NB, dp, dpart);
 	NR3D_LAUNCH_CHECK();
 	return 0;
 }
```

Measured after the change: 1144 Mpoints/s, median of 6. +3.1%, better.
